# RomanJuranek/librectify

Measured on AMD Instinct MI355X. Metric: Mpix/s end-to-end (detect+VP) on 4K frames, batch call of 64 frames, 5 in flight, higher is better.
Workload: dtype f32

## Files before the change

librectify_amd/csrc/batch.hip:

```cpp
#include "host.h"

#include <cstdio>
#include <cstdlib>
#include <cstring>
#include <string>

namespace lramd {

static int find_groups_batch(lr_context* c, const void* d_images_, int format, size_t image_stride, const void* const* h_frames_,
                             int batch, int w, int h, int stride, float min_length, bool refine, int num_threads,
                             LineSegment* out, int capacity, int* n_lines, const RectificationConfig* cfg,
                             ImageTransform* transforms) {
    if (batch <= 0) return 0;
    const uint8_t* d_images = static_cast<const uint8_t*>(d_images_);
    const uint8_t* const* h_frames = reinterpret_cast<const uint8_t* const*>(h_frames_);
    const size_t bpp = (size_t)pix_bytes(format);
    if (bpp == 0) {
        set_error("unknown pixel format of the frames");
        return 1;
    }
    const int S = std::max(1, std::min(c->opt.batch_streams, batch));
    while ((int)c->workers.size() < S - 1) {
        lr_context* wc = nullptr;
        if (ctx_create(c->device, &wc)) return 1;
        c->workers.push_back(wc);
    }
    std::vector<lr_context*> lanes;
    lanes.push_back(c);
    for (int i = 0; i < S - 1; ++i) lanes.push_back(c->workers[i]);
    for (lr_context* l : lanes) {
        l->opt = c->opt;
        l->flood_log_min = S == 1 ? 0 : 32;
        l->flood_log_walk = S == 1 ? 0 : 24;
        l->flood_logbig_off = S > 1;
        l->flood_jit_sleep_us = S == 1 ? 0 : 20;
        static const bool sleep_env = std::getenv("LIBRECTIFY_LANES_SLEEP") != nullptr;
        l->sleep_in_wait = sleep_env && h_frames != nullptr;
    }
    const size_t npix = (size_t)w * h;
    int R = 0;
    bool any_pageable = false;
    std::vector<char> locked(h_frames ? (size_t)batch : 0, 0);
    if (h_frames) {
        if (w < 1 || h < 1) {
            set_error("upload: bad frame");
            return 1;
        }
        if ((stride < 0 ? -stride : stride) < w) {
            set_error("upload: |stride| smaller than the width");
            return 1;
        }
        for (int i = 0; i < batch; ++i) {
            if (h_frames[i] == nullptr) {
                set_error("upload: bad frame");
                return 1;
            }
        }
        for (int i = 0; i < batch; ++i) {
            locked[(size_t)i] = is_page_locked(h_frames[i]);
            any_pageable = any_pageable || !locked[(size_t)i];
        }
        static const int extra_env = std::getenv("LIBRECTIFY_RING_EXTRA") ? std::max(1, std::atoi(std::getenv("LIBRECTIFY_RING_EXTRA"))) : 0;
        const int by_bytes = (int)std::min<size_t>(64, ((size_t)2 << 30) / (npix * bpp));
        R = extra_env ? S + extra_env : std::max(S + 1, std::min(S + 6, by_bytes));
        R = std::min(batch, R);
        if (ensure_upload_ring(c, R, npix, any_pageable)) return 1;
    }
    std::vector<std::atomic<int>> enq(h_frames ? (size_t)batch : 0);
    std::vector<std::atomic<int>> slot_busy((size_t)R);
    struct SlotEdges {
        int r_lo = 0, r_hi = 0;
    };
    std::vector<SlotEdges> slot_edges((size_t)R);
    for (auto& a : enq) a.store(0, std::memory_order_relaxed);
    for (auto& a : slot_busy) a.store(0, std::memory_order_relaxed);
    static const bool lane_debug = std::getenv("LIBRECTIFY_LANE_DEBUG") != nullptr;
    constexpr size_t kBatchBand = (size_t)4 << 20;
    std::atomic<int> abort_all{0};
    std::string up_err;
    auto nap = [](int& spins) {
        if (++spins < 64) std::this_thread::yield();
        else std::this_thread::sleep_for(std::chrono::microseconds(30));
    };
    static const bool batch_stats = std::getenv("LIBRECTIFY_BATCH_STATS") != nullptr;
    std::atomic<long long> up_wait_us{0}, lane_wait_us{0}, lead_sum_us{0};
    std::atomic<int> late_frames{0};
    static const int register_threads = std::getenv("LIBRECTIFY_REGISTER_FRAMES") ? std::max(0, std::atoi(std::getenv("LIBRECTIFY_REGISTER_FRAMES"))) : 4;
    if (c->register_slow_calls > 0) --c->register_slow_calls;
    const bool reg_frames = register_threads > 0 && h_frames != nullptr && any_pageable && stride >= w && c->register_slow_calls == 0;
    const size_t row_bytes = (size_t)w * bpp, pitch = (size_t)(stride < 0 ? -stride : stride) * bpp;
    struct RegPlan {
        uintptr_t lo = 0, hi = 0;
        int r_lo = 0, r_hi = 0;
    };
    std::vector<RegPlan> plan(reg_frames ? (size_t)batch : 0);
    if (reg_frames) {
        constexpr uintptr_t kPage = 4096;
        for (int i = 0; i < batch; ++i) {
            RegPlan& p = plan[(size_t)i];
            const uintptr_t a = reinterpret_cast<uintptr_t>(h_frames[i]), e = a + (size_t)(h - 1) * pitch + row_bytes;
            const uintptr_t lo = (a + kPage - 1) / kPage * kPage, hi = e / kPage * kPage;
            if (hi <= lo) continue;
            const int r_lo = (int)((lo - a + pitch - 1) / pitch);
            const int r_hi = hi - a >= row_bytes ? (int)std::min<size_t>((size_t)h, (hi - a - row_bytes) / pitch + 1) : 0;
            if (r_hi - r_lo < h / 2) continue;
            bool apart = !locked[(size_t)i] && !c->batch_no_register;
            for (int j = 0; j < i && apart; ++j) {
                const RegPlan& q = plan[(size_t)j];
                apart = q.hi <= q.lo || q.hi <= lo || hi <= q.lo;
            }
            if (!apart) continue;
            p.lo = lo;
            p.hi = hi;
            p.r_lo = r_lo;
            p.r_hi = r_hi;
        }
    }
    std::atomic<int> reg_slow{0};
    std::vector<std::atomic<int>> reg_ready(reg_frames ? (size_t)batch : 0);
    for (auto& a : reg_ready) a.store(0, std::memory_order_relaxed);
    std::atomic<int> reg_next{0};
    std::vector<std::thread> reg_pool;
    if (reg_frames)
        for (int t = 0; t < register_threads; ++t)
            reg_pool.emplace_back([&]() {
                (void)hipSetDevice(c->device);
                bind_this_thread_near(c->device);
                for (int i = reg_next.fetch_add(1, std::memory_order_relaxed); i < batch && !abort_all.load(std::memory_order_relaxed);
                     i = reg_next.fetch_add(1, std::memory_order_relaxed)) {
                    if (reg_slow.load(std::memory_order_relaxed) >= 2) break;
                    int expect = 0;
                    if (!reg_ready[(size_t)i].compare_exchange_strong(expect, 3, std::memory_order_acq_rel)) continue;
                    int ok = 2;
                    const double t_r0 = now_ms();
                    const RegPlan& p = plan[(size_t)i];
                    if (p.hi > p.lo)
                        ok = hipHostRegister(reinterpret_cast<void*>(p.lo), p.hi - p.lo, hipHostRegisterDefault) == hipSuccess ? 1 : 2;
                    if (ok == 2) (void)hipGetLastError();
                    if (ok == 1 && (now_ms() - t_r0) * 6.0e6 > (double)(p.hi - p.lo)) reg_slow.fetch_add(1, std::memory_order_relaxed);
                    reg_ready[(size_t)i].store(ok, std::memory_order_release);
                }
            });
    const double t_call0 = now_ms();
    auto uploader = [&]() {
        if (hipSetDevice(c->device) != hipSuccess) {
            up_err = "hipSetDevice failed";
            abort_all.store(1);
            return;
        }
        if (any_pageable) bind_this_thread_near(c->device);
        StagingCrew crew;
        if (any_pageable) crew.start(c, staging_threads(num_threads, npix * bpp) - 1);
        for (int i = 0; i < batch; ++i) {
            int slot = -1, spins = 0;
            const double t_w0 = batch_stats ? now_ms() : 0.0;
            while (slot < 0 && !abort_all.load(std::memory_order_relaxed)) {
                for (int k = 0; k < R && slot < 0; ++k)
                    if (!slot_busy[(size_t)k].load(std::memory_order_acquire)) slot = k;
                if (slot < 0) nap(spins);
            }
            if (batch_stats) up_wait_us.fetch_add((long long)((now_ms() - t_w0) * 1e3));
            if (abort_all.load(std::memory_order_relaxed)) return;
            slot_busy[(size_t)slot].store(1, std::memory_order_relaxed);
            if (reg_frames) {
                int sp2 = 0;
                int expect = 0;
                if (!reg_ready[(size_t)i].compare_exchange_strong(expect, 2, std::memory_order_acq_rel))
                    while (reg_ready[(size_t)i].load(std::memory_order_acquire) == 3 && !abort_all.load(std::memory_order_relaxed)) nap(sp2);
            }
            const bool registered = reg_frames && reg_ready[(size_t)i].load(std::memory_order_acquire) == 1;
            uint8_t* stage = locked[(size_t)i] ? nullptr : reinterpret_cast<uint8_t*>(c->ring.stage[(size_t)slot].get());
            uint8_t* dimg = reinterpret_cast<uint8_t*>(c->ring.img[(size_t)slot].get());
            const double t_u0 = now_ms();
            Event e_dbg;
            if (lane_debug && e_dbg.create() == hipSuccess) (void)hipEventRecord(e_dbg, c->copy_stream);
            int up_rc = 0;
            if (registered) {
                const RegPlan& p = plan[(size_t)i];
                const uint8_t* f = h_frames[i];
                for (int r = 0; r < p.r_lo; ++r) std::memcpy(stage + (size_t)r * row_bytes, f + (size_t)r * pitch, row_bytes);
                for (int r = p.r_hi; r < h; ++r) std::memcpy(stage + (size_t)r * row_bytes, f + (size_t)r * pitch, row_bytes);
                slot_edges[(size_t)slot].r_lo = p.r_lo;
                slot_edges[(size_t)slot].r_hi = p.r_hi;
                {
                    const hipError_t e = pitch == row_bytes
                        ? hipMemcpyAsync(dimg + (size_t)p.r_lo * row_bytes, f + (size_t)p.r_lo * pitch, (size_t)(p.r_hi - p.r_lo) * row_bytes, hipMemcpyHostToDevice, c->copy_stream)
                        : hipMemcpy2DAsync(dimg + (size_t)p.r_lo * row_bytes, row_bytes, f + (size_t)p.r_lo * pitch, pitch, row_bytes, (size_t)(p.r_hi - p.r_lo), hipMemcpyHostToDevice, c->copy_stream);
                    if (e != hipSuccess) up_rc = 1;
                }
                if (up_rc) {
                    (void)hipGetLastError();
                    set_error("upload: transfer of a registered frame failed");
                }
            } else {
                slot_edges[(size_t)slot].r_hi = 0;
                up_rc = stage ? crew.run(dimg, stage, h_frames[i], w, h, stride, (int)bpp, c->copy_stream, kBatchBand, 1)
                              : upload_rows(c, dimg, nullptr, h_frames[i], w, h, stride, (int)bpp, 1, c->copy_stream);
            }
            if (up_rc || hipEventRecord(c->ring_ev[(size_t)slot], c->copy_stream) != hipSuccess) {
                up_err = get_error().empty() ? "upload failed" : get_error();
                abort_all.store(1);
                return;
            }
            enq[(size_t)i].store(slot + 1, std::memory_order_release);
            if (lane_debug) {
                const double t_u1 = now_ms();
                float dma = 0.f;
                if (e_dbg) {
                    (void)hipEventSynchronize(c->ring_ev[(size_t)slot]);
                    if (hipEventElapsedTime(&dma, e_dbg, c->ring_ev[(size_t)slot]) != hipSuccess) (void)hipGetLastError();
                }
                std::fprintf(stderr, "uploader frame %d: slot %d, waited %d naps for it, staged and enqueued in %.2f ms, on the link %.2f ms\n", i, slot, spins, t_u1 - t_u0, dma);
            }
        }
    };
    std::atomic<int> next_frame{0};
    std::vector<int> rc(S, 0);
    std::vector<std::string> err(S);
    auto work = [&](int si) {
        lr_context* l = lanes[si];
        auto fail = [&]() {
            rc[si] = 1;
            err[si] = get_error();
            abort_all.store(1);
        };
        if (si > 0 && hipSetDevice(c->device) != hipSuccess) {
            set_error("hipSetDevice failed");
            return fail();
        }
        for (int b = next_frame.fetch_add(1, std::memory_order_relaxed); b < batch; b = next_frame.fetch_add(1, std::memory_order_relaxed)) {
            const void* img = nullptr;
            int img_stride = stride, slot = -1;
            if (h_frames) {
                int spins = 0;
                const double t_w0 = batch_stats ? now_ms() : 0.0;
                while ((slot = enq[(size_t)b].load(std::memory_order_acquire) - 1) < 0 && !abort_all.load(std::memory_order_relaxed)) nap(spins);
                if (batch_stats) lane_wait_us.fetch_add((long long)((now_ms() - t_w0) * 1e3));
                if (slot < 0) return;
                if (hipStreamWaitEvent(l->stream, c->ring_ev[(size_t)slot], 0) != hipSuccess) {
                    set_error("hipStreamWaitEvent failed");
                    return fail();
                }
                img = c->ring.img[(size_t)slot].get();
                img_stride = w;
                const SlotEdges ed = slot_edges[(size_t)slot];
                if (ed.r_hi > 0) {
                    uint8_t* dimg = reinterpret_cast<uint8_t*>(c->ring.img[(size_t)slot].get());
                    const uint8_t* st = reinterpret_cast<const uint8_t*>(c->ring.stage[(size_t)slot].get());
                    hipError_t e = hipSuccess;
                    if (ed.r_lo > 0) e = hipMemcpyAsync(dimg, st, (size_t)ed.r_lo * row_bytes, hipMemcpyHostToDevice, l->stream);
                    if (e == hipSuccess && ed.r_hi < h)
                        e = hipMemcpyAsync(dimg + (size_t)ed.r_hi * row_bytes, st + (size_t)ed.r_hi * row_bytes, (size_t)(h - ed.r_hi) * row_bytes, hipMemcpyHostToDevice, l->stream);
                    if (e != hipSuccess) {
                        (void)hipGetLastError();
                        set_error("upload: transfer of a registered frame's first or last rows failed");
                        return fail();
                    }
                }
            } else {
                img = d_images + (size_t)b * image_stride * bpp;
            }
            std::vector<LineSegment> res;
            const double t_f0 = now_ms();
            if (ctx_find_groups_device(l, img, format, w, h, img_stride, min_length, refine, res)) return fail();
            if (batch_stats && h_frames && l->opt.timing_on) {
                float lead = 0.f;
                if (hipEventElapsedTime(&lead, c->ring_ev[(size_t)slot], l->ev[0]) == hipSuccess) {
                    lead_sum_us.fetch_add((long long)(lead * 1e3));
                    if (lead < 0.05f) late_frames.fetch_add(1);
                } else {
                    (void)hipGetLastError();
                }
            }
            if (lane_debug) {
                float lead = 0.f;
                if (h_frames && hipEventElapsedTime(&lead, c->ring_ev[(size_t)slot], l->ev[0]) != hipSuccess) (void)hipGetLastError();
                std::fprintf(stderr, "lane %d frame %d: enqueue %.2f ms, wait %.2f, whole call %.2f; device total %.2f; upload done %.2f ms before the first kernel\n",
                             si, b, l->host_ms[0], l->host_ms[2], now_ms() - t_f0, l->stage_ms[LR_T_TOTAL], lead);
            }
            if (h_frames) slot_busy[(size_t)slot].store(0, std::memory_order_release);
            const int n = (int)res.size();
            if (n_lines) n_lines[b] = n;
            if (out && capacity > 0)
                std::memcpy(out + (size_t)b * capacity, res.data(), sizeof(LineSegment) * (size_t)std::min(n, capacity));
            if (transforms) {
                const RectificationConfig def;
                transforms[b] = rectification_transform(res.data(), std::min(n, capacity > 0 ? capacity : n), w, h,
                                                        cfg ? *cfg : def);
            }
        }
    };
    std::vector<std::thread> th;
    if (h_frames) th.emplace_back(uploader);
    for (int si = 1; si < S; ++si) th.emplace_back(work, si);
    work(0);
    for (auto& t : th) t.join();
    if (batch_stats && h_frames)
        std::fprintf(stderr, "batch of %d frames: %.2f ms; the uploader waited %.2f ms for free device frames; the %d lanes waited %.2f ms in all for their frame's transfer to be enqueued\n",
                     batch, now_ms() - t_call0, up_wait_us.load() * 1e-3, S, lane_wait_us.load() * 1e-3);
    if (batch_stats && h_frames && c->opt.timing_on)
        std::fprintf(stderr, "   a frame's transfer was finished %.3f ms (mean) before its first kernel started; %d of %d frames started within 0.05 ms of it (they waited for the link)\n",
                     lead_sum_us.load() * 1e-3 / batch, late_frames.load(), batch);
    if (h_frames) (void)hipStreamSynchronize(c->copy_stream);
    for (auto& t : reg_pool) t.join();
    if (reg_slow.load() >= 2) c->register_slow_calls = 32;
    if (reg_frames)
        for (int i = 0; i < batch; ++i)
            if (reg_ready[(size_t)i].load(std::memory_order_acquire) == 1 && hipHostUnregister(reinterpret_cast<void*>(plan[(size_t)i].lo)) != hipSuccess)
                (void)hipGetLastError();
    for (lr_context* l : lanes) l->sleep_in_wait = false;
    c->flood_logbig_off = false;
    c->flood_log_min = c->flood_log_walk = 0;
    c->flood_jit_sleep_us = 0;
    for (int si = 0; si < S; ++si)
        if (rc[si]) {
            set_error(err[si]);
            return 1;
        }
    if (abort_all.load()) {
        set_error(up_err.empty() ? "batch: upload failed" : up_err);
        return 1;
    }
    return 0;
}

int ctx_find_groups_batch_device(lr_context* c, const void* d_images, int format, size_t image_stride, int batch, int w, int h,
                                 int stride, float min_length, bool refine, LineSegment* out, int capacity, int* n_lines,
                                 const RectificationConfig* cfg, ImageTransform* transforms) {
    return find_groups_batch(c, d_images, format, image_stride, nullptr, batch, w, h, stride, min_length, refine, -1, out,
                             capacity, n_lines, cfg, transforms);
}

int ctx_find_groups_batch_host(lr_context* c, const void* const* frames, int format, int batch, int w, int h, int stride,
                               float min_length, bool refine, int num_threads, LineSegment* out, int capacity,
                               int* n_lines, const RectificationConfig* cfg, ImageTransform* transforms) {
    return find_groups_batch(c, nullptr, format, 0, frames, batch, w, h, stride, min_length, refine, num_threads, out, capacity,
                             n_lines, cfg, transforms);
}

int ctx_find_groups_batch_host_multi(lr_context* c, const int* devices, int n_devices, const void* const* frames, int format, int batch,
                                     int w, int h, int stride, float min_length, bool refine, int num_threads,
                                     LineSegment* out, int capacity, int* n_lines, const RectificationConfig* cfg,
                                     ImageTransform* transforms) {
    if (batch <= 0) return 0;
    if (n_devices <= 0 || devices == nullptr) {
        set_error("multi-device batch: empty device list");
        return 1;
    }
    int ndev = 0;
    if (hipGetDeviceCount(&ndev) != hipSuccess) ndev = 0;
    for (int i = 0; i < n_devices; ++i)
        if (devices[i] < 0 || devices[i] >= ndev) {
            set_error("multi-device batch: device index out of range");
            return 1;
        }
    if ((int)c->peers.size() > n_devices) {
        for (size_t i = (size_t)n_devices; i < c->peers.size(); ++i) ctx_destroy(c->peers[i]);
        c->peers.resize((size_t)n_devices);
    }
    c->peers.resize((size_t)n_devices, nullptr);
    for (int i = 0; i < n_devices; ++i) {
        if (c->peers[(size_t)i] && c->peers[(size_t)i]->device != devices[i]) {
            ctx_destroy(c->peers[(size_t)i]);
            c->peers[(size_t)i] = nullptr;
        }
        if (!c->peers[(size_t)i] && ctx_create(devices[i], &c->peers[(size_t)i])) {
            (void)hipSetDevice(c->device);
            return 1;
        }
        c->peers[(size_t)i]->opt = c->opt;
    }
    const int per = (batch + n_devices - 1) / n_devices;
    bool blocks_apart = true;
    if (const size_t fbpp = (size_t)pix_bytes(format)) {
        const size_t span = (size_t)(h - 1) * (size_t)(stride < 0 ? -stride : stride) * fbpp + (size_t)w * fbpp;
        for (int i = 0; i < batch && blocks_apart && w > 0 && h > 0; ++i)
            for (int j = (i / per + 1) * per; j < batch && blocks_apart; ++j) {
                if (!frames[i] || !frames[j]) continue;
                const uintptr_t a = reinterpret_cast<uintptr_t>(frames[i]) - (stride < 0 ? (size_t)(h - 1) * (size_t)(-stride) * fbpp : 0);
                const uintptr_t b = reinterpret_cast<uintptr_t>(frames[j]) - (stride < 0 ? (size_t)(h - 1) * (size_t)(-stride) * fbpp : 0);
                blocks_apart = a + span <= b || b + span <= a;
            }
    }
    for (lr_context* p : c->peers) p->batch_no_register = !blocks_apart;
    std::vector<int> rc((size_t)n_devices, 0);
    std::vector<std::string> err((size_t)n_devices);
    auto run = [&](int i) {
        const int b0 = std::min(batch, i * per), b1 = std::min(batch, b0 + per);
        if (b1 <= b0) return;
        lr_context* p = c->peers[(size_t)i];
        if (hipSetDevice(p->device) != hipSuccess) {
            rc[(size_t)i] = 1;
            err[(size_t)i] = "hipSetDevice failed";
            return;
        }
        const int nt = num_threads > 1 ? std::max(2, num_threads / std::min(n_devices, (batch + per - 1) / per)) : num_threads;
        if (ctx_find_groups_batch_host(p, frames + b0, format, b1 - b0, w, h, stride, min_length, refine, nt,
                                       out ? out + (size_t)b0 * capacity : nullptr, capacity, n_lines ? n_lines + b0 : nullptr, cfg,
                                       transforms ? transforms + b0 : nullptr)) {
            rc[(size_t)i] = 1;
            err[(size_t)i] = get_error();
        }
    };
    std::vector<std::thread> th;
    for (int i = 1; i < n_devices; ++i) th.emplace_back(run, i);
    run(0);
    for (auto& t : th) t.join();
    (void)hipSetDevice(c->device);
    for (int i = 0; i < n_devices; ++i)
        if (rc[(size_t)i]) {
            set_error("device list entry " + std::to_string(i) + " (device " + std::to_string(devices[i]) + "): " + err[(size_t)i]);
            return 1;
        }
    return 0;
}

}
```

librectify_amd/csrc/common.h:

```cpp
#pragma once
#include <hip/hip_runtime.h>

#include <cstdint>
#include <string>

#include "../../include/librectify_amd.h"

namespace lramd {

constexpr float kEps = 1e-6f;
constexpr int kMaxModels = 4;
constexpr int kMaxPeelModels = 5;
constexpr float kInlierDeg = 2.0f;
constexpr float kGarbageDeg = 4.0f;
constexpr int kRansacMaxIter = 10000;
constexpr int kEdgeKernelSize = 2;
constexpr float kEdgeKernelSigma = 1.0f;
constexpr int kSeedDist = 2;
constexpr float kSeedRatio = 0.95f;
constexpr float kTraceTolerance = 0.25f;
constexpr float kLineMaxErr = 2.0f;
constexpr float kLineMinLength = 5.f;
constexpr int kComponentMinSize = 5;
constexpr int kBins = 8;

struct FilterConsts {
    float d[5];
    float g[5];
    float st[kBins];
    float ct[kBins];
};

struct BinTrig {
    float st[kBins];
    float ct[kBins];
};

constexpr uint32_t kLabelFree = 0xFFFFFFFFu;

__host__ __device__ inline float directional(float dx, float dy, float s, float c) {
    return fabsf(fmaf(dx, s, dy * c));
}

__host__ __device__ inline uint64_t splitmix64(uint64_t x) {
    x += 0x9E3779B97F4A7C15ull;
    x = (x ^ (x >> 30)) * 0xBF58476D1CE4E5B9ull;
    x = (x ^ (x >> 27)) * 0x94D049BB133111EBull;
    return x ^ (x >> 31);
}
__host__ __device__ inline void sample_pair(uint64_t seed, uint32_t round, uint32_t iter, uint32_t n, uint32_t& a,
                                            uint32_t& b) {
    const uint64_t z = splitmix64(seed ^ splitmix64(((uint64_t)round << 32) | iter));
    const uint32_t u1 = (uint32_t)z, u2 = (uint32_t)(z >> 32);
    const uint32_t i = (uint32_t)(((uint64_t)u1 * n) >> 32);
    uint32_t j = (uint32_t)(((uint64_t)u2 * (n - 1)) >> 32);
    if (j >= i) ++j;
    a = i < j ? i : j;
    b = i < j ? j : i;
}

void set_error(const std::string& msg);

#define LR_HIP(expr)                                                                                     \
    do {                                                                                                 \
        hipError_t _e = (expr);                                                                          \
        if (_e != hipSuccess) {                                                                          \
            (void)hipGetLastError();        \
            ::lramd::set_error(std::string(#expr) + ": " + hipGetErrorString(_e) + " (" + __FILE__ + ":" + \
                               std::to_string(__LINE__) + ")");                                          \
            return 1;                                                                                    \
        }                                                                                                \
    } while (0)

inline int pix_bytes(int format) { return format == LR_PIX_U8 ? 1 : format == LR_PIX_U8X3 ? 3 : format == LR_PIX_F32 ? 4 : 0; }
int launch_filter(const void* img, int format, int w, int h, int stride, const FilterConsts& fc, float* dx, float* dy,
                  uint8_t* dmask, uint64_t* cand, uint32_t* cand_count, uint32_t* tile_max, hipStream_t s);
int filter_band_rows();
int filter_band_last_row(int by);
int launch_filter_rows(const void* img, int format, int w, int h, int stride, const FilterConsts& fc, float* dx, float* dy,
                       uint8_t* dmask, uint64_t* cand, uint32_t* cand_count, uint32_t* tile_max, int by_begin, int by_end,
                       hipStream_t s);
struct FilterGeom {
    int n_tiles;
    int cand_cap;
};
FilterGeom filter_geometry(int w, int h);

size_t seeds_temp_bytes(int n_tiles, size_t max_seeds);
int launch_seed_select(const uint64_t* cand, const uint32_t* cand_count, const uint32_t* tile_max, int n_tiles,
                       int cand_cap, float seed_keep_ratio, float* maxmag, uint32_t* tile_pass, uint32_t* tile_off, uint64_t* keys,
                       uint32_t key_cap, uint32_t* n_seeds, uint32_t frame_tag, hipStream_t s);
int launch_seed_order(uint64_t* keys, uint64_t* keys_alt, const uint32_t* n_seeds, uint32_t cap, const float* dx, const float* dy,
                      BinTrig trig, float trace_tolerance, int32_t* seed_idx, int32_t* seed_bin, float* seed_thr, hipStream_t s);

int launch_label_init(uint32_t* label, size_t n, hipStream_t s);
int launch_flood_ordered(const float* dx, const float* dy, const uint8_t* dmask, int w, int h, const int32_t* seed_idx,
                         const int32_t* seed_bin, const float* seed_thr, const uint32_t* d_n_seeds, uint32_t seed_cap,
                         BinTrig trig, uint32_t* label, int32_t* seed_size, int32_t* queue, hipStream_t s);

constexpr size_t kFloodHandWords = 1024;
struct FloodBuffers {
    uint32_t* blocked = nullptr;
    uint32_t* count = nullptr;
    uint32_t* flags = nullptr;
    uint8_t* state = nullptr;
    uint8_t* tier = nullptr;
    uint32_t* blk = nullptr;
    uint32_t* act_a = nullptr;
    uint32_t* act_b = nullptr;
    uint32_t* ctrl = nullptr;
    uint8_t* dirty = nullptr;
    uint32_t* big_list = nullptr;
    uint32_t* handover = nullptr;
    bool rewalk_logs = false;
    uint32_t* rewalk_list = nullptr;
    int log_min_tiles = 0, log_walk_tiles = 0;
    bool giant_hold = false;
    bool giant_step = true;
    void* giant_mask = nullptr;
    uint32_t* giant_parent = nullptr;
    bool log_sweep = false;
    bool rewalk_big = false;
    uint32_t log_seeds = 0, log_cap = 0;
    uint32_t* log_off = nullptr;
    uint32_t* log_len = nullptr;
    uint32_t* log_buf = nullptr;
    void* slab_ring = nullptr;
    void* slab_hash = nullptr;
    uint32_t n_slabs = 0, slab_ring_cap = 0, slab_hash_cap = 0;
    int win_first_shift = 0, win_growth = 2;
    int win_hold_pct = 80;
    bool partial_commits = true;
    bool second_tier = true;
    bool second_tier_from_start = true;
    bool hold_from_start = false;
    bool staged_from_start = false;
    int blind_rounds = 10;
    uint32_t* host_progress = nullptr;
    bool calm_hint = false;
    uint32_t* host_ctrl = nullptr;
    int jit_first = 0;
    int jit_sleep_us = 0;
    uint32_t big_cap_override = 0;
    uint32_t team_tile_cap = 0;
};
struct FloodFrame {
    const float* dx;
    const float* dy;
    const uint8_t* dmask;
    int w, h;
    const int32_t* seed_idx;
    const int32_t* seed_bin;
    const float* seed_thr;
    const uint32_t* d_n_seeds;
    uint32_t seed_cap;
    BinTrig trig;
    uint32_t* label;
    int32_t* seed_size;
    int32_t* queue;
};
struct FloodProgress {
    int enqueued = 0;
    bool use_big = false;
    int win_growth = 2;
    bool sizes_known = false;
    uint32_t max_flood = 0;
};
constexpr int kFloodCtrlWords = 56;
int flood_enqueue(const FloodBuffers& B, const FloodFrame& F, FloodProgress* P, uint32_t* h_ctrl, hipStream_t s);
int flood_finish(const FloodBuffers& B, const FloodFrame& F, FloodProgress* P, uint32_t* h_ctrl, int* rounds_out,
                 uint32_t* tiers_out ,
                 bool* extra, hipStream_t s);

size_t fit_temp_bytes(size_t max_pixels, uint32_t max_segments);
struct HugeSort {
    uint32_t* tab = nullptr;
    uint32_t* list = nullptr;
    uint32_t* jobs = nullptr;
    uint32_t max = 0;
};
int launch_component_offsets(const int32_t* seed_size, const uint32_t* d_n_seeds, uint32_t seed_cap, int min_size,
                             uint32_t* comp_rank, uint32_t* comp_seed, uint32_t* comp_off,
                             uint32_t* totals , uint32_t* large_list, uint32_t large_cap,
                             uint32_t* n_large, void* temp, size_t temp_bytes, uint32_t frame_tag, uint32_t* cursor, const HugeSort& hs,
                             hipStream_t s);
int launch_component_scatter(const uint32_t* label, size_t npix, const uint32_t* comp_rank, const uint32_t* comp_off,
                             uint32_t* cursor, uint32_t* px, const HugeSort& hs, uint32_t* n_large, bool with_huge, hipStream_t s);
int launch_component_sort(const uint32_t* px_in, uint32_t* px_out, const uint32_t* comp_off, const uint32_t* d_n_comp,
                          uint32_t comp_cap, const uint32_t* large_list, uint32_t large_cap, const uint32_t* n_large,
                          uint32_t* scratch, const uint32_t* cursor, const HugeSort& hs, bool with_huge, hipStream_t s);
int launch_fit(const uint32_t* px_sorted, const uint32_t* px_unsorted, const uint32_t* comp_off, const uint32_t* comp_seed, const uint32_t* d_n_comp,
               uint32_t comp_cap, const int32_t* seed_bin, const float* dx, const float* dy, int w, BinTrig trig,
               float* scratch_w, LineSegment* out, const uint32_t* cursor, const HugeSort& hs, const uint32_t* n_large, bool with_huge,
               hipStream_t s);

struct PencilSoA {
    const float* ax;
    const float* ay;
    const float* dx;
    const float* dy;
    const float* len;
    const float* hx;
    const float* hy;
    const float* hz;
};
constexpr int kRansacBestSlots = 32;
int launch_ransac_score(PencilSoA m, uint32_t n, float tol, float degeneracy_tol, uint32_t n_iter, uint64_t seed,
                        uint32_t round, unsigned long long* best_slots, uint32_t* host_best, hipStream_t s);
int launch_ransac_score_dev(PencilSoA m, const uint32_t* gctl, int max_models, float tol, float degeneracy_tol,
                            uint32_t n_iter, uint64_t seed, unsigned long long* best_slots, hipStream_t s);

struct PencilTable {
    float* ax;
    float* ay;
    float* dx;
    float* dy;
    float* len;
    float* hx;
    float* hy;
    float* hz;
    uint32_t* orig;
    PencilSoA soa() const { return PencilSoA{ax, ay, dx, dy, len, hx, hy, hz}; }
};
enum {
    kGcLines = 0,
    kGcRemaining = 1,
    kGcRound = 2,
    kGcActive = 3,
    kGcBestIter0 = 4,
    kGcWords = 8,
};
int launch_filter_lines(const LineSegment* raw, const uint32_t* d_n_raw, uint32_t raw_cap, float min_length,
                        LineSegment* out, uint32_t* gctl, float* gnorm, const PencilTable* all, const PencilTable* round0,
                        hipStream_t s);
int launch_lines_bbox(LineSegment* lines, uint32_t n, uint32_t* gctl, float* gnorm, hipStream_t s);
int launch_pencil_model(const LineSegment* lines, const uint32_t* gctl, const float* gnorm, PencilTable all,
                        PencilTable round0, uint32_t line_cap, hipStream_t s);
int launch_peel(PencilTable cur, PencilTable nxt, PencilTable all, unsigned long long* best_slots, uint64_t seed,
                float tol, float garbage_tol, int max_models, uint32_t* gctl, float* stage4 ,
                LineSegment* lines, float* models,
                const uint32_t* counts, uint32_t cap_lines, void* gather_block ,
                hipStream_t s);
int launch_cht_accumulate(PencilSoA m, uint32_t n, int d, unsigned long long* acc, hipStream_t s);
int launch_cht_votes(PencilSoA m, const uint32_t* idx, uint32_t n, int d, unsigned long long* acc, bool subtract,
                     unsigned long long* n_votes, hipStream_t s);
int launch_cht_peak(const unsigned long long* acc, int d, uint32_t* out3, hipStream_t s);
int launch_refine_pairs(const void* seg, uint32_t n, void* edges, uint32_t* n_edges, uint32_t cap, hipStream_t s);
int launch_prosac_count(PencilSoA m, uint32_t n, float tol, float degeneracy_tol, const uint32_t* sa,
                        const uint32_t* sb, uint32_t n_hyp, uint32_t* counts, hipStream_t s);
int launch_prosac_flags(PencilSoA m, uint32_t n, float px, float py, float pz, float tol, uint8_t* flags, hipStream_t s);
int launch_prosac_records(PencilSoA m, uint32_t n, const uint32_t* sa, const uint32_t* sb, const uint32_t* counts,
                          uint32_t n_hyp, uint32_t best_in, float tol, uint32_t* rec, uint32_t cap, uint8_t* flags, hipStream_t s);
int launch_ht_weights(PencilSoA m, uint32_t n, const int32_t* pa, const int32_t* pb, int n_pairs, int ht, float* peak,
                      float* weights, hipStream_t s);

}
```

librectify_amd/csrc/context.hip:

```cpp
#include "host.h"

#include <cmath>
#include <cstdlib>

#ifndef M_PI
#define M_PI 3.14159265358979323846
#endif

lr_context::lr_context() = default;
lr_context::~lr_context() = default;

namespace lramd {

namespace {

thread_local std::string g_error;

void gauss_deriv_factors(int size, float sigma, float* d, float* g) {
    const int n = 2 * size + 1;
    for (int t = 0; t < n; ++t) {
        const float x = float(t - size);
        const float a = float(2 * M_PI * std::pow(sigma, 4.0f));
        const float e = std::exp(-std::pow(x, 2.0f) / (2 * std::pow(sigma, 2.0f)));
        d[t] = x / a * e;
        g[t] = e;
    }
}

void init_constants(lr_context* c) {
    gauss_deriv_factors(kEdgeKernelSize, kEdgeKernelSigma, c->fconsts.d, c->fconsts.g);
    for (int b = 0; b < kBins; ++b) {
        const float theta = float(b * M_PI) / kBins;
        c->trig.st[b] = std::sin(theta);
        c->trig.ct[b] = std::cos(theta);
        c->fconsts.st[b] = c->trig.st[b];
        c->fconsts.ct[b] = c->trig.ct[b];
    }
    c->seed_keep_ratio = 1 - std::max(std::min(kSeedRatio, 1.f), 0.f);
}

}

void set_error(const std::string& msg) { g_error = msg; }
const std::string& get_error() { return g_error; }

int ctx_trim(lr_context* c, bool frames_too) {
    LR_HIP(hipSetDevice(c->device));
    LR_HIP(hipStreamSynchronize(c->stream));
    if (c->copy_stream) LR_HIP(hipStreamSynchronize(c->copy_stream));
    c->ws = Workspace{};
    c->flood = FloodStore{};
    if (frames_too) {
        c->frames = FrameSlots{};
        c->ring.drop();
        c->prep = PrepareSpans{};
    }
    c->small_frames = 0;
    c->w = c->h = 0;
    c->seed_cap = 0;
    c->flood_hold_hint = c->flood_staged_hint = c->flood_calm_hint = false;
    c->flood_staged_streak = 0;
    for (bool& v : c->stage_valid) v = false;
    if (frames_too)
        for (lr_context* wc : c->workers)
            if (ctx_trim(wc, true)) return 1;
    return 0;
}

int ctx_ensure_image_capacity(lr_context* c, int w, int h) {
    const size_t npix = (size_t)w * h;
    if (c->w != 0 && (c->w != w || c->h != h)) {
        c->flood_hold_hint = false;
        c->flood_staged_hint = false;
        c->flood_calm_hint = false;
        c->flood_staged_streak = 0;
    }
    const FilterGeom fg = filter_geometry(w, h);
    const int ntiles = fg.n_tiles;
    if (c->ws.cap_pix != 0 && npix * 4 <= c->ws.cap_pix) {
        if (++c->small_frames >= 8 && ctx_trim(c, false)) return 1;
    } else {
        c->small_frames = 0;
    }
    if (npix <= c->ws.cap_pix && ntiles <= c->ws.cap_tiles) return 0;
    LR_HIP(hipStreamSynchronize(c->stream));
    const size_t cp = std::max(npix, c->ws.cap_pix);
    const int ct = std::max(ntiles, c->ws.cap_tiles);
    const size_t tile_off_words = std::max(ct, 2);
    Workspace& s = c->ws;
    s.cap_pix = 0;
    s.cap_tiles = 0;
    if (s.dx.grow(cp) || s.dy.grow(cp) || s.dmask.grow(cp + 16) || s.cand.grow((size_t)ct * fg.cand_cap) || s.cand_count.grow(ct) ||
        s.tile_max.grow(ct) || s.tile_pass.grow(ct) || s.tile_off.grow(tile_off_words) || s.keys_a.grow(cp) || s.keys_b.grow(cp) ||
        s.seed_idx.grow(cp) || s.seed_bin.grow(cp) || s.seed_thr.grow(cp) || s.seed_size.grow(cp) || s.label.grow(cp) ||
        s.queue.grow(cp) || s.comp_rank.grow(cp) || s.comp_seed.grow(cp) || s.comp_off.grow(cp + 1) || s.cursor.grow(cp) ||
        s.px_a.grow(cp) || s.px_b.grow(cp) || s.scratch_w.grow(cp) || s.d_lines.grow(cp / 6 + 16) || s.comp_large.grow(cp / 64 + 16))
        return 1;
    LR_HIP(hipMemsetAsync(s.tile_off, 0, tile_off_words * sizeof(uint32_t), c->stream));
    {
        const size_t nb = (cp + 16383) >> 14;
        const uint32_t max = 256;
        if (s.huge_tab.grow(max * nb) || s.huge_jobs.grow(4 * max * nb) || s.huge_list.grow(max)) return 1;
        s.huge = HugeSort{s.huge_tab, s.huge_list, s.huge_jobs, max};
        LR_HIP(hipMemsetAsync(s.huge.tab, 0, max * nb * sizeof(uint32_t), c->stream));
    }
    const size_t tb = std::max(seeds_temp_bytes(ct, cp), fit_temp_bytes(cp, (uint32_t)std::min<size_t>(cp / 6 + 16, 0xFFFFFFFFu)));
    if (s.temp.grow(tb)) return 1;
    LR_HIP(hipMemsetAsync(s.temp, 0, tb, c->stream));
    s.cap_pix = cp;
    s.cap_tiles = ct;
    return 0;
}

template <class T, class P>
static int grow_into(DeviceBuffer<T>& own, P*& raw, size_t count) {
    raw = nullptr;
    if (own.grow(count)) return 1;
    raw = own.get();
    return 0;
}

static int ensure_flood_slabs(lr_context* c) {
    FloodBuffers& f = c->flood.fb;
    static const bool giant_step_off = std::getenv("LIBRECTIFY_FLOOD_GIANT_STEP") && std::atoi(std::getenv("LIBRECTIFY_FLOOD_GIANT_STEP")) == 0;
    uint32_t want = (c->opt.flood_mode == 1 && c->opt.flood_giant_step && !giant_step_off) ? 16u : 128u;
    if (const char* e = std::getenv("LIBRECTIFY_FLOOD_SLABS")) want = (uint32_t)std::max(1, std::atoi(e));
    if (f.slab_ring && f.n_slabs >= want) return 0;
    LR_HIP(hipStreamSynchronize(c->stream));
    f.n_slabs = want;
    f.slab_ring_cap = 1u << 14;
    f.slab_hash_cap = 1u << 16;
    if (grow_into(c->flood.slab_ring, f.slab_ring, (size_t)f.n_slabs * f.slab_ring_cap) ||
        grow_into(c->flood.slab_hash, f.slab_hash, (size_t)f.n_slabs * f.slab_hash_cap * 2))
        return 1;
    LR_HIP(hipMemsetAsync(f.slab_hash, 0, (size_t)f.n_slabs * f.slab_hash_cap * 32, c->stream));
    if (f.ctrl) LR_HIP(hipMemsetAsync(f.ctrl, 0, kFloodCtrlWords * sizeof(uint32_t), c->stream));
    return 0;
}

int ensure_flood_buffers(lr_context* c) {
    FloodStore& o = c->flood;
    FloodBuffers& f = o.fb;
    if (c->flood.cap_seeds >= c->ws.cap_pix && f.ctrl) return ensure_flood_slabs(c);
    LR_HIP(hipStreamSynchronize(c->stream));
    const size_t cs = c->ws.cap_pix;
    if (grow_into(o.blocked, f.blocked, cs) || grow_into(o.count, f.count, cs) || grow_into(o.flags, f.flags, cs) ||
        grow_into(o.state, f.state, cs) || grow_into(o.tier, f.tier, cs) || grow_into(o.blk, f.blk, cs) ||
        grow_into(o.act_a, f.act_a, cs) || grow_into(o.act_b, f.act_b, cs) || grow_into(o.ctrl, f.ctrl, kFloodCtrlWords) ||
        grow_into(o.big_list, f.big_list, 8192) || grow_into(o.handover, f.handover, 8192 * kFloodHandWords) ||
        grow_into(o.dirty, f.dirty, cs / 256 + 16) ||
        grow_into(o.giant_mask, f.giant_mask, cs / 16 + 64))
        return 1;
    constexpr size_t kLogCapDiv = 8;
    f.log_seeds = (uint32_t)std::min<size_t>(std::max<size_t>(cs / 16, 4096), cs);
    f.log_cap = (uint32_t)std::min<size_t>(std::max<size_t>(cs / kLogCapDiv, 65536), 1u << 28);
    if (grow_into(o.rewalk_list, f.rewalk_list, 8192) || grow_into(o.log_off, f.log_off, f.log_seeds) ||
        grow_into(o.log_len, f.log_len, f.log_seeds) || grow_into(o.log_buf, f.log_buf, (size_t)f.log_cap * 3))
        return 1;
    LR_HIP(hipMemsetAsync(f.ctrl, 0, kFloodCtrlWords * sizeof(uint32_t), c->stream));
    o.cap_seeds = cs;
    return ensure_flood_slabs(c);
}


int ctx_ensure_ransac_capacity(lr_context* c, size_t n_lines) {
    if (8 * n_lines <= c->model.cap()) return 0;
    LR_HIP(hipStreamSynchronize(c->stream));
    return c->model.grow(8 * std::max<size_t>(n_lines, 4096));
}

int ensure_group_capacity(lr_context* c, size_t n_lines) {
    if (n_lines > c->cap_glines) {
        LR_HIP(hipStreamSynchronize(c->stream));
        const size_t cl = std::max<size_t>(n_lines, 4096);
        c->cap_glines = 0;
        if (c->d_tables.grow(3 * 8 * cl) || c->d_orig.grow(3 * cl) || c->d_inl.grow(4 * cl)) return 1;
        c->cap_glines = cl;
    }
    if (n_lines > c->d_flines.cap()) {
        LR_HIP(hipStreamSynchronize(c->stream));
        if (c->d_flines.grow(n_lines + 16)) return 1;
    }
    return 0;
}

int ctx_create(int device, lr_context** out) {
    int ndev = 0;
    if (hipGetDeviceCount(&ndev) != hipSuccess || ndev <= 0) {
        set_error("no HIP device available: librectify_amd has no CPU fallback");
        return 1;
    }
    if (device < 0 || device >= ndev) {
        set_error("device index out of range");
        return 1;
    }
    LR_HIP(hipSetDevice(device));
    lr_context* c = new lr_context();
    c->device = device;
    if (hipStreamCreateWithFlags(c->stream.put(), hipStreamNonBlocking) != hipSuccess) {
        delete c;
        set_error("hipStreamCreate failed");
        return 1;
    }
    {
        static const int fail_at = std::getenv("LIBRECTIFY_TEST_CREATE_FAIL") ? std::atoi(std::getenv("LIBRECTIFY_TEST_CREATE_FAIL")) : 0;
        int n_alloc = 0;
        hipError_t bad = hipSuccess;
        const char* what = "";
        auto check = [&](hipError_t e, const char* name) {
            if (++n_alloc == fail_at) e = hipErrorOutOfMemory;
            if (e != hipSuccess && bad == hipSuccess) {
                bad = e;
                what = name;
            }
        };
        for (auto& e : c->ev) check(e.create(), "hipEventCreate");
        check(c->ev_wait.create(hipEventBlockingSync | hipEventDisableTiming), "hipEventCreate");
        static const bool lane_debug = std::getenv("LIBRECTIFY_LANE_DEBUG") != nullptr;
        for (auto& e : c->ev_up) check(e.create(lane_debug ? hipEventDefault : hipEventDisableTiming), "hipEventCreate");
        check(c->maxmag.alloc(1), "hipMalloc(maxmag)");
        check(c->d_counts.alloc(64), "hipMalloc(counts)");
        check(c->d_gctl.alloc(kGcWords), "hipMalloc(peeling control block)");
        check(c->d_gnorm.alloc(4), "hipMalloc(normalisation)");
        check(c->d_models.alloc(64), "hipMalloc(models)");
        check(c->d_best_slots.alloc(kRansacBestSlots), "hipMalloc(best slots)");
        check(c->h_counts.alloc(128), "hipHostMalloc(counts)");
        check(c->h_best.alloc(2), "hipHostMalloc(best)");
        if (bad == hipSuccess) check(hipMemset(c->d_models, 0, 64 * sizeof(float)), "hipMemset(models)");
        if (bad == hipSuccess) check(hipMemset(c->d_counts, 0, 64 * sizeof(uint32_t)), "hipMemset(counts)");
        if (bad == hipSuccess) check(hipMemset(c->d_best_slots, 0, kRansacBestSlots * sizeof(unsigned long long)), "hipMemset(best slots)");
        if (bad != hipSuccess) {
            (void)hipGetLastError();
            const std::string msg = std::string("lr_context_create: ") + what + " failed: " + hipGetErrorString(bad);
            ctx_destroy(c);
            set_error(msg);
            return 1;
        }
    }
    init_constants(c);
    const char* env = std::getenv("LIBRECTIFY_SEED");
    c->opt.ransac_seed = env ? std::strtoull(env, nullptr, 0) : 0ull;
    c->opt.timing_on = std::getenv("LIBRECTIFY_STAGE_TIMES") != nullptr;
    if (const char* e = std::getenv("LIBRECTIFY_FLOOD_LOGS")) c->opt.flood_logs = std::atoi(e) != 0;
    *out = c;
    return 0;
}

void ctx_destroy(lr_context* c) {
    if (!c) return;
    for (lr_context* wc : c->workers) ctx_destroy(wc);
    for (lr_context* pc : c->peers) ctx_destroy(pc);
    (void)hipSetDevice(c->device);
    (void)hipStreamSynchronize(c->stream);
    if (c->copy_stream) (void)hipStreamSynchronize(c->copy_stream);
    c->crew.reset();
    delete c;
}

}
```

librectify_amd/csrc/frame.hip:

```cpp
#include "host.h"

#include <cstdio>
#include <cstdlib>
#include <cstring>

namespace lramd {


namespace {

uint32_t round_up(uint32_t v, uint32_t m) { return (v + m - 1) / m * m; }

uint32_t initial_seed_cap(size_t npix) {
    return (uint32_t)std::min<size_t>(npix, std::max<size_t>(round_up((uint32_t)(npix / 32), 1024), 4096));
}

uint32_t line_cap_for(const lr_context* c) {
    return (uint32_t)std::min<size_t>(c->seed_cap, c->ws.cap_pix / 6 + 16);
}


PencilTable table_of(lr_context* c, int which) {
    const size_t cl = c->cap_glines;
    float* b = c->d_tables + (size_t)which * 8 * cl;
    return PencilTable{b, b + cl, b + 2 * cl, b + 3 * cl, b + 4 * cl, b + 5 * cl, b + 6 * cl, b + 7 * cl,
                       c->d_orig + (size_t)which * cl};
}

int ensure_result_block(lr_context* c, size_t lines) {
    if (lines <= c->res_lines_cap && c->h_res) return 0;
    LR_HIP(hipStreamSynchronize(c->stream));
    if (c->h_res.grow(kResHeaderBytes + lines * sizeof(LineSegment))) return 1;
    c->res_lines_cap = lines;
    return 0;
}

FloodBuffers flood_buffers_for(lr_context* c) {
    FloodBuffers fbuf = c->flood.fb;
    if (c->opt.flood_mode >= 2 && c->opt.flood_mode <= 4) fbuf.second_tier = false;
    fbuf.second_tier_from_start = c->flood_big_hint;
    fbuf.hold_from_start = c->flood_hold_hint;
    fbuf.staged_from_start = c->flood_staged_hint;
    if (c->opt.flood_mode == 2) fbuf.n_slabs = 0;
    if (c->opt.flood_mode == 3) fbuf.n_slabs = 2;
    if (c->opt.flood_mode == 5) {
        fbuf.n_slabs = 0;
        fbuf.big_cap_override = 1;
    }
    if (c->opt.flood_mode == 6) fbuf.team_tile_cap = 200;
    if (c->opt.flood_mode == 7) {
        fbuf.team_tile_cap = 200;
        fbuf.n_slabs = 0;
    }
    static const bool partial_off = std::getenv("LIBRECTIFY_FLOOD_PARTIAL") && std::atoi(std::getenv("LIBRECTIFY_FLOOD_PARTIAL")) == 0;
    fbuf.partial_commits = !partial_off && c->opt.flood_partial;
    fbuf.rewalk_logs = c->opt.flood_logs;
    fbuf.log_sweep = c->opt.flood_log_sweep;
    fbuf.log_min_tiles = c->flood_log_min;
    fbuf.log_walk_tiles = c->flood_log_walk;
    fbuf.giant_hold = c->opt.flood_mode == 1;
    static const bool giant_step_off = std::getenv("LIBRECTIFY_FLOOD_GIANT_STEP") && std::atoi(std::getenv("LIBRECTIFY_FLOOD_GIANT_STEP")) == 0;
    fbuf.giant_step = !giant_step_off && c->opt.flood_giant_step;
    fbuf.giant_parent = reinterpret_cast<uint32_t*>(c->ws.queue.get());
    fbuf.rewalk_big = c->flood_logbig_hint && !c->flood_logbig_off;
    if (c->opt.flood_staged) fbuf.win_first_shift = 3;
    fbuf.blind_rounds = c->flood_rounds_hint;
    static const bool jit_off = std::getenv("LIBRECTIFY_FLOOD_JIT") && std::atoi(std::getenv("LIBRECTIFY_FLOOD_JIT")) == 0;
    static_assert(16 + kFloodCtrlWords <= 72, "the control block's copy ends where the report word begins");
    fbuf.host_progress = c->h_counts + 72;
    fbuf.host_ctrl = c->h_counts + 16;
    static const int calm_hint_env = std::getenv("LIBRECTIFY_FLOOD_CALM_HINT") ? std::atoi(std::getenv("LIBRECTIFY_FLOOD_CALM_HINT")) : 1;
    fbuf.calm_hint = calm_hint_env != 0 && c->flood_calm_hint;
    fbuf.jit_sleep_us = c->flood_jit_sleep_us;
    constexpr int kJitFirstMax = 4;
    fbuf.jit_first = (c->opt.flood_jit && !jit_off) ? std::min(c->flood_rounds_last > 0 ? std::max(c->flood_rounds_last - 1, 2) : 3, kJitFirstMax) : 0;
    return fbuf;
}

FloodFrame flood_frame_for(lr_context* c) {
    return FloodFrame{c->ws.dx, c->ws.dy, c->ws.dmask, c->w, c->h, c->ws.seed_idx, c->ws.seed_bin, c->ws.seed_thr,
                      c->d_counts + kCntSeeds, c->seed_cap, c->trig, c->ws.label, c->ws.seed_size, c->ws.queue};
}

int prepare_frame(lr_context* c, int w, int h) {
    LR_HIP(hipSetDevice(c->device));
    if (w < 5 || h < 5) {
        set_error("image smaller than the 5x5 filter");
        return 1;
    }
    if (ctx_ensure_image_capacity(c, w, h)) return 1;
    if (c->w != w || c->h != h || c->seed_cap == 0) c->seed_cap = initial_seed_cap((size_t)w * h);
    if (c->seed_cap_once) {
        c->seed_cap = (uint32_t)std::min<size_t>((size_t)w * h, c->seed_cap_once);
        c->seed_cap_once = 0;
    }
    c->w = w;
    c->h = h;
    c->n_seeds = c->n_comp = c->n_px = 0;
    c->dmask_consumed = false;
    for (bool& v : c->stage_valid) v = false;
    return 0;
}

int enqueue_filter(lr_context* c, const void* d_image, int format, int w, int h, int stride) {
    if (prepare_frame(c, w, h)) return 1;
    const size_t bpp = (size_t)pix_bytes(format);
    if (bpp == 0 || d_image == nullptr || stride < w) {
        set_error(bpp == 0 ? "unknown pixel format of the frames" : "launch_filter: bad geometry");
        return 1;
    }
    const size_t npix = (size_t)w * h;
    if (format == LR_PIX_U8X3) {
        if (npix >= ((size_t)1 << 29)) {
            set_error("launch_filter: image larger than 2^29 pixels is not supported (seed key packs index in 29 bits)");
            return 1;
        }
        if (c->frames.luma.cap() < npix) {
            LR_HIP(hipStreamSynchronize(c->stream));
            if (c->frames.luma.grow(npix)) return 1;
        }
        if (ctx_prepare_frames(c, d_image, 0, 1, w, h, (size_t)stride * bpp, LR_PIX_U8X3, c->frames.luma.get(), 0, w, h, (size_t)w * sizeof(float)))
            return 1;
        d_image = c->frames.luma.get();
        format = LR_PIX_F32;
        stride = w;
    }
    const size_t fbpp = (size_t)pix_bytes(format);
    if (stride > w && (uint64_t)w * (uint64_t)h < (1ull << 29) &&
        ((uint64_t)(h - 1) * (uint64_t)stride + (uint64_t)w) * fbpp >= (1ull << 32)) {
        if (c->frames.packed.cap() < npix) {
            LR_HIP(hipStreamSynchronize(c->stream));
            if (c->frames.packed.grow(npix)) return 1;
        }
        LR_HIP(hipMemcpy2DAsync(c->frames.packed, (size_t)w * fbpp, d_image, (size_t)stride * fbpp,
                                (size_t)w * fbpp, (size_t)h, hipMemcpyDeviceToDevice, c->stream));
        d_image = c->frames.packed;
        stride = w;
    }
    if (c->opt.timing_on) LR_HIP(hipEventRecord(c->ev[0], c->stream));
    if (launch_filter(d_image, format, w, h, stride, c->fconsts, c->ws.dx, c->ws.dy, c->ws.dmask, c->ws.cand, c->ws.cand_count, c->ws.tile_max,
                      c->stream))
        return 1;
    if (c->opt.timing_on) LR_HIP(hipEventRecord(c->ev[1], c->stream));
    return 0;
}

int enqueue_seeds(lr_context* c) {
    const FilterGeom fg = filter_geometry(c->w, c->h);
    if (launch_seed_select(c->ws.cand, c->ws.cand_count, c->ws.tile_max, fg.n_tiles, fg.cand_cap, c->seed_keep_ratio, c->maxmag,
                           c->ws.tile_pass, c->ws.tile_off, c->ws.keys_a, c->seed_cap, c->d_counts + kCntSeeds, ++c->select_tag ? c->select_tag : ++c->select_tag,
                           c->stream))
        return 1;
    if (launch_seed_order(c->ws.keys_a, c->ws.keys_b, c->d_counts + kCntSeeds, c->seed_cap, c->ws.dx, c->ws.dy, c->trig, kTraceTolerance,
                          c->ws.seed_idx, c->ws.seed_bin, c->ws.seed_thr, c->stream))
        return 1;
    if (c->opt.timing_on) LR_HIP(hipEventRecord(c->ev[2], c->stream));
    return 0;
}

int enqueue_flood(lr_context* c) {
    const size_t npix = (size_t)c->w * c->h;
    c->flood_rounds = 1;
    if (c->opt.flood_mode == 0) {
        if (launch_label_init(c->ws.label, npix, c->stream)) return 1;
        if (launch_flood_ordered(c->ws.dx, c->ws.dy, c->ws.dmask, c->w, c->h, c->ws.seed_idx, c->ws.seed_bin, c->ws.seed_thr,
                                 c->d_counts + kCntSeeds, c->seed_cap, c->trig, c->ws.label, c->ws.seed_size, c->ws.queue, c->stream))
            return 1;
    } else {
        if (ensure_flood_buffers(c)) return 1;
        if (flood_enqueue(flood_buffers_for(c), flood_frame_for(c), &c->flood_prog, c->h_counts + 16, c->stream)) return 1;
        c->stage_valid[0] = c->stage_valid[1] = false;
        c->dmask_consumed = true;
    }
    if (c->opt.timing_on) LR_HIP(hipEventRecord(c->ev[3], c->stream));
    return 0;
}

int finish_flood(lr_context* c, bool* extra) {
    *extra = false;
    if (c->opt.flood_mode == 0) return 0;
    if (flood_finish(flood_buffers_for(c), flood_frame_for(c), &c->flood_prog, c->h_counts + 16, &c->flood_rounds,
                     c->flood_tiers, extra, c->stream))
        return 1;
    static const bool call_debug = std::getenv("LIBRECTIFY_CALL_DEBUG") != nullptr;
    if (call_debug)
        std::fprintf(stderr, "flood: %d rounds, %u walks in the second tier, %u of them long, hold-back phase %u (started with it: %d)\n",
                     c->flood_rounds, c->flood_tiers[0], c->flood_tiers[8], c->flood_tiers[3], (int)c->flood_hold_hint);
    c->flood_logbig_hint = c->flood_tiers[0] > 0;
    c->flood_calm_hint = c->flood_tiers[0] == 0 && c->flood_tiers[1] == 0 && c->flood_tiers[15] == 0;
    c->flood_big_hint = true;
    c->flood_hold_hint = c->flood_tiers[3] != 0 && c->flood_tiers[8] >= 16;
    constexpr uint32_t kStagedKeep = 64;
    c->flood_staged_hint = c->flood_tiers[14] != 0 && (!c->flood_staged_hint || c->flood_tiers[0] >= kStagedKeep);
    c->flood_staged_streak = c->flood_staged_hint ? c->flood_staged_streak + 1 : 0;
    if (c->flood_staged_streak >= 16) {
        c->flood_staged_hint = false;
        c->flood_staged_streak = 0;
    }
    if (c->flood_staged_hint) c->flood_hold_hint = false;

    c->flood_rounds_hint = std::max(std::max(c->flood_rounds + 2, 6), c->flood_rounds_hint - 1);
    c->flood_rounds_last = c->flood_rounds;
    return 0;
}

int enqueue_fit(lr_context* c) {
    const size_t npix = (size_t)c->w * c->h;
    const uint32_t comp_cap = line_cap_for(c);
    const bool with_huge = !(c->opt.flood_mode != 0 && c->flood_prog.sizes_known && c->flood_prog.max_flood <= (1u << 14));
    if (launch_component_offsets(c->ws.seed_size, c->d_counts + kCntSeeds, c->seed_cap, kComponentMinSize, c->ws.comp_rank,
                                 c->ws.comp_seed, c->ws.comp_off, c->d_counts + kCntComp, c->ws.comp_large,
                                 (uint32_t)(c->ws.cap_pix / 64 + 16), c->d_counts + kCntLarge, c->ws.temp, c->ws.temp.cap(), ++c->fit_tag ? c->fit_tag : ++c->fit_tag, c->ws.cursor,
                                 with_huge ? c->ws.huge : HugeSort{}, c->stream))
        return 1;
    if (launch_component_scatter(c->ws.label, npix, c->ws.comp_rank, c->ws.comp_off, c->ws.cursor, c->ws.px_a, c->ws.huge, c->d_counts + kCntLarge, with_huge,
                                 c->stream))
        return 1;
    if (launch_component_sort(c->ws.px_a, c->ws.px_b, c->ws.comp_off, c->d_counts + kCntComp, comp_cap, c->ws.comp_large,
                              (uint32_t)(c->ws.cap_pix / 64 + 16), c->d_counts + kCntLarge, reinterpret_cast<uint32_t*>(c->ws.keys_b.get()),
                              c->ws.cursor, c->ws.huge, with_huge, c->stream))
        return 1;
    static const bool fit_debug = std::getenv("LIBRECTIFY_FIT_DEBUG") != nullptr;
    if (fit_debug) {
        uint32_t cnt[16];
        LR_HIP(hipStreamSynchronize(c->stream));
        LR_HIP(hipMemcpy(cnt, c->d_counts, sizeof(cnt), hipMemcpyDeviceToHost));
        std::fprintf(stderr, "fit: with_huge %d (sizes known %d, largest flood %u); seeds %u comps %u px %u; lists: %u of 65..1024 px, %u longer, %u huge in %u buckets; counter %u\n",
                     (int)with_huge, (int)c->flood_prog.sizes_known, c->flood_prog.max_flood, cnt[0], cnt[1], cnt[2], cnt[4], cnt[5], cnt[6], cnt[7], cnt[10]);
        const uint32_t nj = std::min<uint32_t>(cnt[7], 6);
        std::vector<uint32_t> jobs(4 * nj + 4);
        if (nj) LR_HIP(hipMemcpy(jobs.data(), c->ws.huge.jobs, nj * 16, hipMemcpyDeviceToHost));
        for (uint32_t j = 0; j < nj; ++j) std::fprintf(stderr, "   bucket job %u: start %u, %u px, table word %u\n", j, jobs[4 * j], jobs[4 * j + 1], jobs[4 * j + 2]);
    }
    if (launch_fit(c->ws.px_b, c->ws.px_a, c->ws.comp_off, c->ws.comp_seed, c->d_counts + kCntComp, comp_cap, c->ws.seed_bin, c->ws.dx, c->ws.dy, c->w,
                   c->trig, c->ws.scratch_w, c->ws.d_lines, c->ws.cursor, c->ws.huge, c->d_counts + kCntLarge, with_huge, c->stream))
        return 1;
    if (c->opt.timing_on) LR_HIP(hipEventRecord(c->ev[4], c->stream));
    return 0;
}

}

int enqueue_groups(lr_context* c, uint32_t line_cap, int max_models, float inlier_deg, float garbage_deg, int n_iter,
                   uint64_t seed, bool model_done, bool gather) {
    if (max_models > kMaxPeelModels) {
        set_error("estimate_line_pencils: max_models above " + std::to_string(kMaxPeelModels) + " (the reference uses 4, config.h:25)");
        return 1;
    }
    const float tol = cos_threshold(inlier_deg), garbage_tol = cos_threshold(garbage_deg);
    const PencilTable all = table_of(c, 0);
    PencilTable tab[2] = {table_of(c, 1), table_of(c, 2)};
    if (!model_done && launch_pencil_model(c->d_flines, c->d_gctl, c->d_gnorm, all, tab[0], line_cap, c->stream)) return 1;
    const float degeneracy_tol = 0.05f;
    for (int k = 0; k < max_models; ++k) {
        if (n_iter > 0 &&
            launch_ransac_score_dev(tab[k & 1].soa(), c->d_gctl, max_models, tol, degeneracy_tol, (uint32_t)n_iter, seed,
                                    c->d_best_slots, c->stream))
            return 1;
        const bool last = gather && k == max_models - 1;
        if (launch_peel(tab[k & 1], tab[(k + 1) & 1], all, c->d_best_slots, seed, tol, garbage_tol,
                        max_models, c->d_gctl, c->d_inl, c->d_flines, c->d_models, c->d_counts,
                        (uint32_t)std::min<size_t>(c->res_lines_cap, c->d_flines.cap()), last ? c->h_res.get() : nullptr, c->stream))
            return 1;
    }
    return 0;
}

namespace {

void record_stage_times(lr_context* c, bool with_groups) {
    if (!c->opt.timing_on) return;
    float ms = 0.f;
    (void)hipEventElapsedTime(&ms, c->ev[0], c->ev[1]);
    c->stage_ms[LR_T_FILTER] = ms;
    c->stage_ms[LR_T_FILTER_KERNEL] = ms;
    (void)hipEventElapsedTime(&ms, c->ev[1], c->ev[2]);
    c->stage_ms[LR_T_SEEDS] = ms;
    (void)hipEventElapsedTime(&ms, c->ev[2], c->ev[3]);
    c->stage_ms[LR_T_FLOOD] = ms;
    (void)hipEventElapsedTime(&ms, c->ev[3], c->ev[4]);
    c->stage_ms[LR_T_FIT] = ms;
    if (with_groups) {
        (void)hipEventElapsedTime(&ms, c->ev[5], c->ev[6]);
        c->stage_ms[LR_T_RANSAC] = ms;
        (void)hipEventElapsedTime(&ms, c->ev[0], c->ev[6]);
        c->stage_ms[LR_T_TOTAL] = ms;
    }
}

void adapt_seed_cap(lr_context* c, uint32_t n_seeds) {
    const size_t npix = (size_t)c->w * c->h;
    if (n_seeds > c->seed_cap)
        c->seed_cap = (uint32_t)std::min<size_t>(npix, std::max<uint32_t>(4096, round_up(n_seeds * 2u, 1024)));
    else if (n_seeds < c->seed_cap / 3 || n_seeds > c->seed_cap / 5 * 4)
        c->seed_cap = (uint32_t)std::min<size_t>(npix, std::max<uint32_t>(4096, round_up(n_seeds + n_seeds / 2, 1024)));
}

}

struct TimingOn {
    lr_context* c;
    bool was;
    explicit TimingOn(lr_context* ctx) : c(ctx), was(ctx->opt.timing_on) { c->opt.timing_on = true; }
    ~TimingOn() { c->opt.timing_on = was; }
};

int ctx_stage_filter(lr_context* c, const float* d_image, int w, int h, int stride) {
    TimingOn t(c);
    if (enqueue_filter(c, d_image, LR_PIX_F32, w, h, stride)) return 1;
    c->stage_valid[0] = true;
    return 0;
}

int ctx_stage_seeds(lr_context* c) {
    if (!c->stage_valid[0]) {
        set_error("lr_stage_seeds: run lr_stage_filter first");
        return 1;
    }
    TimingOn t(c);
    for (int attempt = 0;; ++attempt) {
        if (enqueue_seeds(c)) return 1;
        LR_HIP(hipMemcpyAsync(c->h_counts, c->d_counts, sizeof(uint32_t), hipMemcpyDeviceToHost, c->stream));
        LR_HIP(hipStreamSynchronize(c->stream));
        c->n_seeds = c->h_counts[0];
        if (c->n_seeds <= c->seed_cap) break;
        if (attempt > 0) {
            set_error("seed count exceeds the sort capacity twice");
            return 1;
        }
        adapt_seed_cap(c, c->n_seeds);
    }
    c->stage_valid[1] = true;
    return 0;
}

int ctx_stage_flood(lr_context* c) {
    if (!c->stage_valid[1]) {
        set_error(c->dmask_consumed ? "lr_stage_flood: the previous flood consumed the filter output; run lr_stage_filter and lr_stage_seeds again"
                                    : "lr_stage_flood: run lr_stage_seeds first");
        return 1;
    }
    TimingOn t(c);
    if (enqueue_flood(c)) return 1;
    LR_HIP(hipStreamSynchronize(c->stream));
    bool extra;
    if (finish_flood(c, &extra)) return 1;
    c->stage_valid[2] = true;
    return 0;
}

int ctx_stage_fit(lr_context* c, std::vector<LineSegment>& out) {
    if (!c->stage_valid[2]) {
        set_error("lr_stage_fit: run lr_stage_flood first");
        return 1;
    }
    out.clear();
    TimingOn t(c);
    if (enqueue_fit(c)) return 1;
    LR_HIP(hipMemcpyAsync(c->h_counts, c->d_counts, 8 * sizeof(uint32_t), hipMemcpyDeviceToHost, c->stream));
    LR_HIP(hipStreamSynchronize(c->stream));
    c->n_comp = c->h_counts[kCntComp];
    c->n_px = c->h_counts[kCntPx];
    if (c->n_comp > 0) {
        out.resize(c->n_comp);
        LR_HIP(hipMemcpyAsync(out.data(), c->ws.d_lines, (size_t)c->n_comp * sizeof(LineSegment), hipMemcpyDeviceToHost,
                              c->stream));
        LR_HIP(hipStreamSynchronize(c->stream));
    }
    c->stage_valid[3] = true;
    record_stage_times(c, false);
    return 0;
}

int ctx_detect(lr_context* c, const float* d_image, int w, int h, int stride, std::vector<LineSegment>& raw) {
    if (ctx_stage_filter(c, d_image, w, h, stride)) return 1;
    if (ctx_stage_seeds(c)) return 1;
    if (ctx_stage_flood(c)) return 1;
    return ctx_stage_fit(c, raw);
}

int run_frame(lr_context* c, const void* d_image, int format, int w, int h, int stride, float min_length, bool refine,
              std::vector<LineSegment>& out, bool filter_enqueued) {
    out.clear();
    const double t_begin = now_ms();
    const bool fused = !refine && c->opt.estimator == 0;
    const int n_iter = c->opt.ransac_iters;
    auto groups_after_fit = [&]() -> int {
        const uint32_t lc = line_cap_for(c);
        if (ensure_group_capacity(c, lc)) return 1;
        if (ensure_result_block(c, std::max<size_t>(c->res_lines_cap, 4096))) return 1;
        if (c->opt.timing_on) LR_HIP(hipEventRecord(c->ev[5], c->stream));
        const PencilTable all = table_of(c, 0), round0 = table_of(c, 1);
        if (launch_filter_lines(c->ws.d_lines, c->d_counts + kCntComp, lc, min_length, c->d_flines, c->d_gctl, c->d_gnorm, &all, &round0,
                                c->stream))
            return 1;
        static_assert(kMaxModels >= 1 && kGcWords == 8 && kResHeaderBytes == 256, "the last peeling round carries the result block (peel_kernel)");
        if (enqueue_groups(c, lc, kMaxModels, kInlierDeg, kGarbageDeg, n_iter, c->opt.ransac_seed, true, true)) return 1;
        if (c->opt.timing_on) LR_HIP(hipEventRecord(c->ev[6], c->stream));
        return 0;
    };
    auto after_fit = [&]() -> int {
        if (fused) return groups_after_fit();
        LR_HIP(hipMemcpyAsync(c->h_counts, c->d_counts, 8 * sizeof(uint32_t), hipMemcpyDeviceToHost, c->stream));
        return 0;
    };
    c->frame_laps = 0;
    for (int attempt = 0;; ++attempt) {
        c->frame_laps += 1;
        if (!(filter_enqueued && attempt == 0) && enqueue_filter(c, d_image, format, w, h, stride)) return 1;
        if (enqueue_seeds(c)) return 1;
        if (enqueue_flood(c)) return 1;
        if (enqueue_fit(c)) return 1;
        if (after_fit()) return 1;
        const double t_enq = now_ms();
        const double t_pre = now_ms();
        if (c->sleep_in_wait) {
            LR_HIP(hipEventRecord(c->ev_wait, c->stream));
            LR_HIP(hipEventSynchronize(c->ev_wait));
        } else {
            LR_HIP(hipStreamSynchronize(c->stream));
        }
        c->host_ms[0] = t_enq - t_begin;
        c->host_ms[1] = t_pre - t_enq;
        c->host_ms[2] = now_ms() - t_pre;
        const uint32_t* cnt = fused ? reinterpret_cast<const uint32_t*>(c->h_res.get()) : c->h_counts.get();
        c->n_seeds = cnt[kCntSeeds];
        if (c->n_seeds <= c->seed_cap) break;
        if (attempt > 0) {
            set_error("seed count exceeds the sort capacity twice");
            return 1;
        }
        adapt_seed_cap(c, c->n_seeds);
    }
    bool extra = false;
    if (finish_flood(c, &extra)) return 1;
    if (extra) {
        c->frame_laps += 1;
        if (enqueue_fit(c)) return 1;
        if (after_fit()) return 1;
        LR_HIP(hipStreamSynchronize(c->stream));
    }
    const uint32_t* cnt = fused ? reinterpret_cast<const uint32_t*>(c->h_res.get()) : c->h_counts.get();
    c->n_comp = cnt[kCntComp];
    c->n_px = cnt[kCntPx];
    adapt_seed_cap(c, c->n_seeds);
    c->stage_valid[0] = c->stage_valid[1] = false;
    c->stage_valid[2] = c->stage_valid[3] = true;
    if (fused) {
        const uint32_t* gctl = reinterpret_cast<const uint32_t*>(c->h_res + 32);
        const size_t n = gctl[kGcLines];
        out.resize(n);
        const size_t have = std::min<size_t>(n, c->res_lines_cap);
        if (have) std::memcpy(out.data(), c->h_res + kResHeaderBytes, have * sizeof(LineSegment));
        if (n > have) {
            LR_HIP(hipMemcpyAsync(out.data() + have, c->d_flines + have, (n - have) * sizeof(LineSegment),
                                  hipMemcpyDeviceToHost, c->stream));
            LR_HIP(hipStreamSynchronize(c->stream));
            if (ensure_result_block(c, round_up((uint32_t)(n + n / 2), 1024))) return 1;
        }
        record_stage_times(c, true);
#ifdef LR_PEEL_TIMING
        {
            const float* tm = reinterpret_cast<const float*>(c->h_res + 64) + 16;
            for (int r = 0; r < 4; ++r)
                std::fprintf(stderr, "peel round %d: best %.1f us, inliers %.1f, sums %.1f, jacobi %.1f, verdict %.1f\n", r,
                             tm[r * 5], tm[r * 5 + 1], tm[r * 5 + 2], tm[r * 5 + 3], tm[r * 5 + 4]);
        }
#endif
        return 0;
    }
    std::vector<LineSegment> raw(c->n_comp);
    if (c->n_comp) {
        LR_HIP(hipMemcpyAsync(raw.data(), c->ws.d_lines, (size_t)c->n_comp * sizeof(LineSegment), hipMemcpyDeviceToHost,
                              c->stream));
        LR_HIP(hipStreamSynchronize(c->stream));
    }
    record_stage_times(c, false);
    if (raw.size() < 2) return 0;
    if (refine && ctx_refine(c, raw)) return 1;
    std::vector<LineSegment> filtered = filter_lines(raw, min_length);
    if (filtered.empty()) return 0;
    if (c->opt.timing_on) LR_HIP(hipEventRecord(c->ev[5], c->stream));
    if (c->opt.estimator == 1) {
        if (ctx_estimate_line_pencils_prosac(c, filtered, kMaxModels, kInlierDeg, kGarbageDeg, c->opt.prosac_T_N,
                                             c->opt.ransac_seed))
            return 1;
    } else if (c->opt.estimator == 2) {
        if (ctx_estimate_line_pencils_direct(c, filtered, kMaxModels, kInlierDeg, kGarbageDeg)) return 1;
    } else if (c->opt.estimator == 3) {
        if (ctx_estimate_line_pencils_cht(c, filtered, kMaxModels, kInlierDeg, kGarbageDeg, c->opt.cht_d, nullptr)) return 1;
    } else if (ctx_estimate_line_pencils(c, filtered, kMaxModels, kInlierDeg, kGarbageDeg, n_iter, c->opt.ransac_seed)) {
        return 1;
    }
    if (c->opt.timing_on) LR_HIP(hipEventRecord(c->ev[6], c->stream));
    LR_HIP(hipStreamSynchronize(c->stream));
    record_stage_times(c, true);
    out.swap(filtered);
    return 0;
}

int ctx_find_groups_device(lr_context* c, const void* d_image, int format, int w, int h, int stride, float min_length, bool refine,
                           std::vector<LineSegment>& out) {
    return run_frame(c, d_image, format, w, h, stride, min_length, refine, out);
}

int ctx_find_groups_host(lr_context* c, const void* buffer_, int format, int w, int h, int stride, float min_length, bool refine,
                         int num_threads, std::vector<LineSegment>& out) {
    const uint8_t* buffer = static_cast<const uint8_t*>(buffer_);
    const int bpp = pix_bytes(format);
    if (bpp == 0) {
        set_error("unknown pixel format of the frames");
        return 1;
    }
    const double t_call = now_ms();
    LR_HIP(hipSetDevice(c->device));
    if (w < 5 || h < 5 || buffer == nullptr) {
        set_error("image smaller than the 5x5 filter");
        return 1;
    }
    if ((stride < 0 ? -stride : stride) < w) {
        set_error("upload: |stride| smaller than the width");
        return 1;
    }
    if (ensure_copy_stream(c)) return 1;
    hipStream_t up = c->copy_stream;
    const size_t npix = (size_t)w * h;
    const int slot = 0;
    uint8_t* stage = nullptr;
    {
        float* stage_f = nullptr;
        if (ensure_frame_slot(c, slot, npix, !is_page_locked(buffer), &stage_f)) return 1;
        stage = reinterpret_cast<uint8_t*>(stage_f);
    }
    if (prepare_frame(c, w, h)) return 1;
    struct DrainOnError {
        lr_context* c;
        hipStream_t up;
        bool ok = false;
        ~DrainOnError() {
            if (ok) return;
            (void)hipStreamSynchronize(up);
            (void)hipStreamSynchronize(c->stream);
            (void)hipGetLastError();
        }
    } drain{c, up};
    const uint8_t* src = buffer;
    int sstride = stride;
    if (sstride < 0) {
        src = buffer + (std::ptrdiff_t)(h - 1) * sstride * bpp;
        sstride = -sstride;
    }
    const size_t row_bytes = (size_t)w * bpp, pitch = (size_t)sstride * bpp;
    const bool follow = format != LR_PIX_U8X3;
    static const size_t band_bytes = std::getenv("LIBRECTIFY_UPLOAD_BAND_KB") ? (size_t)std::max(64, std::atoi(std::getenv("LIBRECTIFY_UPLOAD_BAND_KB"))) << 10 : (size_t)4 << 20;
    static const bool band_env = std::getenv("LIBRECTIFY_UPLOAD_BAND_KB") != nullptr;
    int rpb = (int)std::max<size_t>(1, ((stage == nullptr && !band_env) ? (size_t)h * row_bytes : band_bytes) / row_bytes);
    if ((h + rpb - 1) / rpb > StagingCrew::kMaxBands) rpb = (h + StagingCrew::kMaxBands - 1) / StagingCrew::kMaxBands;
    const int n_bands = (h + rpb - 1) / rpb;
    while ((int)c->band_ev.size() < n_bands) {
        Event e;
        if (e.ensure(hipEventDisableTiming)) return 1;
        c->band_ev.push_back(std::move(e));
    }
    uint8_t* dst = reinterpret_cast<uint8_t*>(c->frames.slot[slot].get());
    const int fb = filter_band_rows(), band_rows = (h + fb - 1) / fb;
    int by_next = 0;
    auto filter_after_band = [&](int k) -> int {
        LR_HIP(hipStreamWaitEvent(c->stream, c->band_ev[(size_t)k], 0));
        if (!follow) return 0;
        const int last_row = std::min(h, (k + 1) * rpb) - 1;
        int by_end = by_next;
        while (by_end < band_rows && std::min(h - 1, filter_band_last_row(by_end)) <= last_row) ++by_end;
        if (k == n_bands - 1) by_end = band_rows;
        if (launch_filter_rows(dst, format, w, h, w, c->fconsts, c->ws.dx, c->ws.dy, c->ws.dmask, c->ws.cand, c->ws.cand_count, c->ws.tile_max, by_next,
                               by_end, c->stream))
            return 1;
        by_next = by_end;
        return 0;
    };
    if (follow && c->opt.timing_on) LR_HIP(hipEventRecord(c->ev[0], c->stream));
    const int T = stage ? staging_threads(num_threads, npix * bpp) : 1;
    if (T <= 1) {
        for (int k = 0; k < n_bands; ++k) {
            const int r0 = k * rpb, r1 = std::min(h, r0 + rpb);
            if (stage) {
                if (sstride == w) std::memcpy(stage + (size_t)r0 * row_bytes, src + (size_t)r0 * pitch, (size_t)(r1 - r0) * row_bytes);
                else
                    for (int r = r0; r < r1; ++r) std::memcpy(stage + (size_t)r * row_bytes, src + (size_t)r * pitch, row_bytes);
                LR_HIP(hipMemcpyAsync(dst + (size_t)r0 * row_bytes, stage + (size_t)r0 * row_bytes, (size_t)(r1 - r0) * row_bytes,
                                      hipMemcpyHostToDevice, up));
            } else if (sstride == w) {
                LR_HIP(hipMemcpyAsync(dst + (size_t)r0 * row_bytes, src + (size_t)r0 * row_bytes, (size_t)(r1 - r0) * row_bytes,
                                      hipMemcpyHostToDevice, up));
            } else {
                LR_HIP(hipMemcpy2DAsync(dst + (size_t)r0 * row_bytes, row_bytes, src + (size_t)r0 * pitch, pitch,
                                        row_bytes, (size_t)(r1 - r0), hipMemcpyHostToDevice, up));
            }
            LR_HIP(hipEventRecord(c->band_ev[(size_t)k], up));
            if (filter_after_band(k)) return 1;
        }
    } else {
        if (!c->crew || c->crew_helpers != T) {
            c->crew.reset();
            c->crew.reset(new StagingCrew());
            c->crew->start(c, T);
            c->crew_helpers = T;
        }
        StagingCrew* cr = c->crew.get();
        std::vector<std::atomic<int>> ready((size_t)n_bands);
        for (auto& a : ready) a.store(0, std::memory_order_relaxed);
        const uint32_t g = cr->begin(dst, stage, src, w, h, sstride, bpp, up, c->band_ev.data(), ready.data(), band_bytes);
        int rc = 0;
        for (int k = 0; k < n_bands && rc == 0; ++k) {
            int spins = 0, r;
            while ((r = ready[(size_t)k].load(std::memory_order_acquire)) == 0) {
                if ((cr->live.load(std::memory_order_acquire) == 0 || spins > 4096) && cr->work_one(g)) continue;
                if (++spins < 2048) std::this_thread::yield();
                else std::this_thread::sleep_for(std::chrono::microseconds(5));
            }
            if (r < 0 || filter_after_band(k)) rc = 1;
        }
        if (rc) cr->work(g);
        if (cr->finish() || rc) {
            if (get_error().empty()) set_error("upload: staging copy failed");
            return 1;
        }
    }
    if (follow && c->opt.timing_on) LR_HIP(hipEventRecord(c->ev[1], c->stream));
    LR_HIP(hipEventRecord(c->ev_up[slot], up));
    static const bool call_debug = std::getenv("LIBRECTIFY_CALL_DEBUG") != nullptr;
    const double t_up = now_ms();
    const int rc = run_frame(c, dst, format, w, h, w, min_length, refine, out, follow);
    drain.ok = rc == 0;
    if (call_debug)
        std::fprintf(stderr, "host frame: bands staged, sent and filter launched in %.3f ms; rest of the frame enqueued in %.3f ms; waited %.3f ms; "
                     "results out in %.3f ms; whole call %.3f ms\n", t_up - t_call, c->host_ms[0], c->host_ms[2],
                     now_ms() - t_up - c->host_ms[0] - c->host_ms[2], now_ms() - t_call);
    return rc;
}

}
```

librectify_amd/csrc/kernels_groups.hip:

```cpp
#include "common.h"

namespace lramd {
namespace {

constexpr int kWG = 1024;
constexpr int kWaves = kWG / 64;

__device__ __forceinline__ float wave_tree(float v) {
#pragma unroll
    for (int off = 32; off >= 1; off >>= 1) v = v + __shfl_xor(v, off);
    return v;
}

__device__ __forceinline__ uint32_t block_rank(bool flag, uint32_t* s_cnt, uint32_t& total) {
    const int lane = threadIdx.x & 63, wv = threadIdx.x >> 6;
    const uint64_t m = __ballot(flag);
    __syncthreads();
    if (lane == 0) s_cnt[wv] = (uint32_t)__popcll(m);
    __syncthreads();
    uint32_t before = 0, tot = 0;
#pragma unroll
    for (int i = 0; i < kWaves; ++i) {
        const uint32_t c = s_cnt[i];
        before += i < wv ? c : 0u;
        tot += c;
    }
    total = tot;
    return before + (uint32_t)__popcll(m & ((1ull << lane) - 1ull));
}

__device__ __forceinline__ void pencil_model_of(const LineSegment& l, uint32_t i, float cx, float cy, float sc, const PencilTable& all,
                                                const PencilTable& round0) {
    const float x1 = (l.x1 - cx) / sc, y1 = (l.y1 - cy) / sc, x2 = (l.x2 - cx) / sc, y2 = (l.y2 - cy) / sc;
    float hx = y1 * 1.f - 1.f * y2, hy = 1.f * x2 - x1 * 1.f, hz = x1 * y2 - y1 * x2;
    const float zz = (hx * hx + hy * hy) + hz * hz;
    if (zz > 0.0f) {
        const float nn = sqrtf(zz);
        hx = hx / nn;
        hy = hy / nn;
        hz = hz / nn;
    }
    const float ax = (x2 + x1) / 2, ay = (y2 + y1) / 2;
    const float dx = x2 - x1, dy = y2 - y1;
    const float len = sqrtf(dx * dx + dy * dy);
    const float ux = dx / len, uy = dy / len;
    all.ax[i] = ax; all.ay[i] = ay; all.dx[i] = ux; all.dy[i] = uy; all.len[i] = len;
    all.hx[i] = hx; all.hy[i] = hy; all.hz[i] = hz; all.orig[i] = i;
    round0.ax[i] = ax; round0.ay[i] = ay; round0.dx[i] = ux; round0.dy[i] = uy; round0.len[i] = len;
    round0.hx[i] = hx; round0.hy[i] = hy; round0.hz[i] = hz; round0.orig[i] = i;
}

__global__ __launch_bounds__(kWG) void filter_lines_kernel(const LineSegment* __restrict__ raw,
                                                           const uint32_t* __restrict__ n_raw_ptr, uint32_t raw_cap,
                                                           float min_length, LineSegment* __restrict__ out,
                                                           uint32_t* __restrict__ gctl, float* __restrict__ gnorm,
                                                           PencilTable all, PencilTable round0, uint32_t with_model) {
    constexpr int kFlB = 8;
    __shared__ uint32_t s_cnt[kFlB][kWaves];
    __shared__ float s_red[4][kWaves];
    const uint32_t n_raw = min(*n_raw_ptr, raw_cap);
    const float ml = fmaxf(min_length, kLineMinLength);
    const int lane = threadIdx.x & 63, wv = threadIdx.x >> 6;
    uint32_t base = 0;
    if (n_raw >= 2u) {
        for (uint32_t i0 = 0; i0 < n_raw; i0 += kWG * kFlB) {
            LineSegment l[kFlB];
            uint64_t m[kFlB];
#pragma unroll
            for (int b = 0; b < kFlB; ++b) {
                const uint32_t i = i0 + (uint32_t)b * kWG + threadIdx.x;
                l[b] = LineSegment{};
                if (i < n_raw) l[b] = raw[i];
            }
#pragma unroll
            for (int b = 0; b < kFlB; ++b) {
                const uint32_t i = i0 + (uint32_t)b * kWG + threadIdx.x;
                const float dx = l[b].x2 - l[b].x1, dy = l[b].y2 - l[b].y1;
                const bool keep = i < n_raw && sqrtf(dx * dx + dy * dy) > ml && l[b].err < kLineMaxErr;
                m[b] = __ballot(keep);
                if (lane == 0) s_cnt[b][wv] = (uint32_t)__popcll(m[b]);
            }
            __syncthreads();
#pragma unroll
            for (int b = 0; b < kFlB; ++b) {
                uint32_t before = 0, tot = 0;
#pragma unroll
                for (int w = 0; w < kWaves; ++w) {
                    const uint32_t c = s_cnt[b][w];
                    before += w < wv ? c : 0u;
                    tot += c;
                }
                if ((m[b] >> lane) & 1ull) {
                    l[b].group_id = -1;
                    out[base + before + (uint32_t)__popcll(m[b] & ((1ull << lane) - 1ull))] = l[b];
                }
                base += tot;
            }
            __syncthreads();
        }
    }
    __syncthreads();
    const uint32_t n = base;
    float mnx = INFINITY, mny = INFINITY, mxx = -INFINITY, mxy = -INFINITY;
    for (uint32_t i = threadIdx.x; i < n; i += kWG) {
        const LineSegment l = out[i];
        mnx = fminf(mnx, fminf(l.x1, l.x2));
        mny = fminf(mny, fminf(l.y1, l.y2));
        mxx = fmaxf(mxx, fmaxf(l.x1, l.x2));
        mxy = fmaxf(mxy, fmaxf(l.y1, l.y2));
    }
#pragma unroll
    for (int off = 32; off >= 1; off >>= 1) {
        mnx = fminf(mnx, __shfl_xor(mnx, off));
        mny = fminf(mny, __shfl_xor(mny, off));
        mxx = fmaxf(mxx, __shfl_xor(mxx, off));
        mxy = fmaxf(mxy, __shfl_xor(mxy, off));
    }
    if ((threadIdx.x & 63) == 0) {
        s_red[0][threadIdx.x >> 6] = mnx;
        s_red[1][threadIdx.x >> 6] = mny;
        s_red[2][threadIdx.x >> 6] = mxx;
        s_red[3][threadIdx.x >> 6] = mxy;
    }
    __syncthreads();
    if (threadIdx.x == 0) {
        for (int i = 1; i < kWaves; ++i) {
            mnx = fminf(mnx, s_red[0][i]);
            mny = fminf(mny, s_red[1][i]);
            mxx = fmaxf(mxx, s_red[2][i]);
            mxy = fmaxf(mxy, s_red[3][i]);
        }
        const float sx = mxx - mnx, sy = mxy - mny;
        gnorm[0] = mnx + 0.5f * sx;
        gnorm[1] = mny + 0.5f * sy;
        gnorm[2] = fmaxf(sx, sy);
        gctl[kGcLines] = n;
        gctl[kGcRemaining] = n;
        gctl[kGcRound] = 0u;
        gctl[kGcActive] = n;
        s_red[0][0] = gnorm[0];
        s_red[1][0] = gnorm[1];
        s_red[2][0] = gnorm[2];
    }
    if (with_model == 0u) return;
    __syncthreads();
    const float cx = s_red[0][0], cy = s_red[1][0], sc = s_red[2][0];
    for (uint32_t i = threadIdx.x; i < n; i += kWG) pencil_model_of(out[i], i, cx, cy, sc, all, round0);
}

__global__ __launch_bounds__(kWG) void lines_bbox_kernel(LineSegment* __restrict__ lines, uint32_t n,
                                                         uint32_t* __restrict__ gctl, float* __restrict__ gnorm) {
    __shared__ float s_red[4][kWaves];
    float mnx = INFINITY, mny = INFINITY, mxx = -INFINITY, mxy = -INFINITY;
    for (uint32_t i = threadIdx.x; i < n; i += kWG) {
        const LineSegment l = lines[i];
        mnx = fminf(mnx, fminf(l.x1, l.x2));
        mny = fminf(mny, fminf(l.y1, l.y2));
        mxx = fmaxf(mxx, fmaxf(l.x1, l.x2));
        mxy = fmaxf(mxy, fmaxf(l.y1, l.y2));
        lines[i].group_id = -1;
    }
#pragma unroll
    for (int off = 32; off >= 1; off >>= 1) {
        mnx = fminf(mnx, __shfl_xor(mnx, off));
        mny = fminf(mny, __shfl_xor(mny, off));
        mxx = fmaxf(mxx, __shfl_xor(mxx, off));
        mxy = fmaxf(mxy, __shfl_xor(mxy, off));
    }
    if ((threadIdx.x & 63) == 0) {
        s_red[0][threadIdx.x >> 6] = mnx;
        s_red[1][threadIdx.x >> 6] = mny;
        s_red[2][threadIdx.x >> 6] = mxx;
        s_red[3][threadIdx.x >> 6] = mxy;
    }
    __syncthreads();
    if (threadIdx.x == 0) {
        for (int i = 1; i < kWaves; ++i) {
            mnx = fminf(mnx, s_red[0][i]);
            mny = fminf(mny, s_red[1][i]);
            mxx = fmaxf(mxx, s_red[2][i]);
            mxy = fmaxf(mxy, s_red[3][i]);
        }
        const float sx = mxx - mnx, sy = mxy - mny;
        gnorm[0] = mnx + 0.5f * sx;
        gnorm[1] = mny + 0.5f * sy;
        gnorm[2] = fmaxf(sx, sy);
        gctl[kGcLines] = n;
        gctl[kGcRemaining] = n;
        gctl[kGcRound] = 0u;
        gctl[kGcActive] = n;
    }
}

__global__ __launch_bounds__(256) void pencil_model_kernel(const LineSegment* __restrict__ lines,
                                                           const uint32_t* __restrict__ gctl,
                                                           const float* __restrict__ gnorm, PencilTable all,
                                                           PencilTable round0) {
    const uint32_t i = blockIdx.x * 256 + threadIdx.x;
    if (i >= gctl[kGcLines]) return;
    pencil_model_of(lines[i], i, gnorm[0], gnorm[1], gnorm[2], all, round0);
}

__device__ __forceinline__ float pencil_error(float ax, float ay, float dx, float dy, float px, float py, float pz) {
    float vx, vy;
    if (fabsf(pz) < kEps) {
        vx = px;
        vy = py;
    } else {
        const float qx = px / pz, qy = py / pz;
        vx = qx - ax;
        vy = qy - ay;
    }
    const float nn = vx * vx + vy * vy;
    const float nrm = sqrtf(nn);
    const float ux = vx / nrm, uy = vy / nrm;
    return -fabsf(ux * dx + uy * dy) + 1.0f;
}

__device__ void smallest_eigenvector_3x3(const float c[9], float out[3]) {
    double A[3][3];
    double V[3][3] = {{1, 0, 0}, {0, 1, 0}, {0, 0, 1}};
    for (int i = 0; i < 3; ++i)
        for (int j = 0; j < 3; ++j) A[i][j] = 0.5 * ((double)c[i * 3 + j] + (double)c[j * 3 + i]);
    for (int sweep = 0; sweep < 64; ++sweep) {
        const double off = A[0][1] * A[0][1] + A[0][2] * A[0][2] + A[1][2] * A[1][2];
        const double dg = A[0][0] * A[0][0] + A[1][1] * A[1][1] + A[2][2] * A[2][2];
        if (off <= 1e-36 * dg) break;
        for (int p = 0; p < 2; ++p)
            for (int q = p + 1; q < 3; ++q) {
                if (A[p][q] == 0.0) continue;
                const double theta = (A[q][q] - A[p][p]) / (2.0 * A[p][q]);
                const double t = (theta >= 0 ? 1.0 : -1.0) / (fabs(theta) + sqrt(theta * theta + 1.0));
                const double cs = 1.0 / sqrt(t * t + 1.0), sn = t * cs;
                for (int k = 0; k < 3; ++k) {
                    const double akp = A[k][p], akq = A[k][q];
                    A[k][p] = cs * akp - sn * akq;
                    A[k][q] = sn * akp + cs * akq;
                }
                for (int k = 0; k < 3; ++k) {
                    const double apk = A[p][k], aqk = A[q][k];
                    A[p][k] = cs * apk - sn * aqk;
                    A[q][k] = sn * apk + cs * aqk;
                }
                for (int k = 0; k < 3; ++k) {
                    const double vkp = V[k][p], vkq = V[k][q];
                    V[k][p] = cs * vkp - sn * vkq;
                    V[k][q] = sn * vkp + cs * vkq;
                }
            }
    }
    int k = 0;
    if (A[1][1] < A[k][k]) k = 1;
    if (A[2][2] < A[k][k]) k = 2;
    const double nx = V[0][k], ny = V[1][k], nz = V[2][k];
    const double nn = sqrt(nx * nx + ny * ny + nz * nz);
    out[0] = (float)(nx / nn);
    out[1] = (float)(ny / nn);
    out[2] = (float)(nz / nn);
}

constexpr uint32_t kStage = 2048;
__device__ __forceinline__ void peel_body(const PencilTable& cur, const PencilTable& nxt, const PencilTable& all,
                                          unsigned long long* __restrict__ best_slots, uint64_t seed,
                                          float tol, float garbage_tol, int max_models,
                                          uint32_t* __restrict__ gctl, float4* __restrict__ stage_g,
                                          LineSegment* __restrict__ lines, float* __restrict__ models) {
    __shared__ uint32_t s_cnt[kWaves];
    __shared__ float s_bv[kWaves];
    __shared__ int s_bi[kWaves];
    __shared__ float s_h[3];
    __shared__ float4 s_stage[kStage];
    const int lane = threadIdx.x & 63, wv = threadIdx.x >> 6;
    const uint32_t n = gctl[kGcActive];
    const uint32_t round = gctl[kGcRound];
    if (gctl[kGcRemaining] < 2u || round >= (uint32_t)max_models) return;

#ifdef LR_PEEL_TIMING
    unsigned long long tm[6];
    tm[0] = wall_clock64();
#endif
    float r_ax = 0.f, r_ay = 0.f, r_dx = 0.f, r_dy = 0.f, r_len = 0.f, r_hx = 0.f, r_hy = 0.f, r_hz = 0.f;
    uint32_t r_orig = 0;
    if (threadIdx.x < n) {
        const uint32_t i = threadIdx.x;
        r_ax = cur.ax[i]; r_ay = cur.ay[i]; r_dx = cur.dx[i]; r_dy = cur.dy[i]; r_len = cur.len[i];
        r_hx = cur.hx[i]; r_hy = cur.hy[i]; r_hz = cur.hz[i]; r_orig = cur.orig[i];
    }

    if (threadIdx.x < 64) {
        unsigned long long key = threadIdx.x < (unsigned)kRansacBestSlots ? best_slots[threadIdx.x] : 0ull;
        if (threadIdx.x < (unsigned)kRansacBestSlots) best_slots[threadIdx.x] = 0ull;
#pragma unroll
        for (int off = 32; off >= 1; off >>= 1) {
            const unsigned long long o = ((unsigned long long)(uint32_t)__shfl_xor((int)(uint32_t)(key >> 32), off) << 32) |
                                         (uint32_t)__shfl_xor((int)(uint32_t)key, off);
            key = o > key ? o : key;
        }
        if (threadIdx.x == 0) {
            s_bv[0] = __uint_as_float((uint32_t)(key >> 32));
            s_bi[0] = key ? (int)(0xFFFFFFFFu - (uint32_t)key) : -1;
        }
    }
    __syncthreads();
    if (threadIdx.x == 0) {
        const int bi = s_bi[0];
        float hx = 0.f, hy = 0.f, hz = 0.f;
        if (bi >= 0) {
            uint32_t a, b;
            sample_pair(seed, round, (uint32_t)bi, n, a, b);
            const float ax = cur.hx[a], ay = cur.hy[a], az = cur.hz[a];
            const float bx = cur.hx[b], by = cur.hy[b], bz = cur.hz[b];
            hx = ay * bz - az * by;
            hy = az * bx - ax * bz;
            hz = ax * by - ay * bx;
        }
        s_h[0] = hx;
        s_h[1] = hy;
        s_h[2] = hz;
        if (round < (uint32_t)(kGcWords - kGcBestIter0)) gctl[kGcBestIter0 + round] = (uint32_t)bi;
    }
    __syncthreads();
    const float bx_ = s_h[0], by_ = s_h[1], bz_ = s_h[2];
#ifdef LR_PEEL_TIMING
    tm[1] = wall_clock64();
#endif

    uint32_t n_inl = 0;
    for (uint32_t i0 = 0; i0 < n; i0 += kWG) {
        const uint32_t i = i0 + threadIdx.x;
        bool in = false;
        float4 hl = make_float4(r_hx, r_hy, r_hz, r_len);
        if (i < n) {
            if (i0 == 0) {
                in = pencil_error(r_ax, r_ay, r_dx, r_dy, bx_, by_, bz_) < tol;
            } else {
                in = pencil_error(cur.ax[i], cur.ay[i], cur.dx[i], cur.dy[i], bx_, by_, bz_) < tol;
                if (in) hl = make_float4(cur.hx[i], cur.hy[i], cur.hz[i], cur.len[i]);
            }
        }
        uint32_t tot;
        const uint32_t r = block_rank(in, s_cnt, tot);
        if (in) {
            const uint32_t o = n_inl + r;
            if (o < kStage) s_stage[o] = hl;
            else stage_g[o] = hl;
        }
        n_inl += tot;
    }
    __syncthreads();

#ifdef LR_PEEL_TIMING
    tm[2] = wall_clock64();
#endif
    if (wv == 0) {
        const uint32_t m = n_inl ? n_inl : gctl[kGcLines];
        float acc[9];
#pragma unroll
        for (int k = 0; k < 9; ++k) acc[k] = 0.f;
        for (uint32_t j = lane; j < m; j += 64) {
            float4 hl;
            if (n_inl) hl = j < kStage ? s_stage[j] : stage_g[j];
            else hl = make_float4(all.hx[j], all.hy[j], all.hz[j], all.len[j]);
            const float hv[3] = {hl.x, hl.y, hl.z};
#pragma unroll
            for (int a = 0; a < 3; ++a) {
                const float t = hv[a] * hl.w;
#pragma unroll
                for (int b = 0; b < 3; ++b) acc[a * 3 + b] = acc[a * 3 + b] + t * hv[b];
            }
        }
#pragma unroll
        for (int k = 0; k < 9; ++k) acc[k] = wave_tree(acc[k]);
#ifdef LR_PEEL_TIMING
        tm[3] = wall_clock64();
#endif
        if (lane == 0) {
            float hf[3];
            smallest_eigenvector_3x3(acc, hf);
            s_h[0] = hf[0];
            s_h[1] = hf[1];
            s_h[2] = hf[2];
            if (round < (uint32_t)kMaxPeelModels) {
                models[round * 3 + 0] = hf[0];
                models[round * 3 + 1] = hf[1];
                models[round * 3 + 2] = hf[2];
            }
        }
    }
    __syncthreads();
    const float fx = s_h[0], fy = s_h[1], fz = s_h[2];
#ifdef LR_PEEL_TIMING
    tm[4] = wall_clock64();
#endif

    uint32_t n_next = 0, n_gone = 0;
    for (uint32_t i0 = 0; i0 < n; i0 += kWG) {
        const uint32_t i = i0 + threadIdx.x;
        bool stay = false, gone = false;
        if (i < n) {
            if (i0 != 0) {
                r_ax = cur.ax[i]; r_ay = cur.ay[i]; r_dx = cur.dx[i]; r_dy = cur.dy[i]; r_len = cur.len[i];
                r_hx = cur.hx[i]; r_hy = cur.hy[i]; r_hz = cur.hz[i]; r_orig = cur.orig[i];
            }
            const float e = pencil_error(r_ax, r_ay, r_dx, r_dy, fx, fy, fz);
            if (e < tol) {
                lines[r_orig].group_id = (int)round;
                gone = true;
            } else if (e >= tol && e < garbage_tol) {
                gone = true;
            } else {
                stay = true;
            }
        }
        uint32_t tot, tg;
        const uint32_t r = block_rank(stay, s_cnt, tot);
        if (stay) {
            const uint32_t o = n_next + r;
            nxt.ax[o] = r_ax; nxt.ay[o] = r_ay; nxt.dx[o] = r_dx; nxt.dy[o] = r_dy;
            nxt.len[o] = r_len; nxt.hx[o] = r_hx; nxt.hy[o] = r_hy; nxt.hz[o] = r_hz;
            nxt.orig[o] = r_orig;
        }
        (void)block_rank(gone, s_cnt, tg);
        n_next += tot;
        n_gone += tg;
    }
#ifdef LR_PEEL_TIMING
    if (threadIdx.x == 0) {
        tm[5] = wall_clock64();
        for (int q = 0; q < 5 && round < 4u; ++q) models[16 + round * 5 + q] = (float)(tm[q + 1] - tm[q]) * 0.01f;
    }
#endif
    if (threadIdx.x == 0) {
        gctl[kGcActive] = n_next;
        gctl[kGcRemaining] = gctl[kGcRemaining] - n_gone;
        gctl[kGcRound] = round + 1u;
    }
}

__global__ __launch_bounds__(kWG) void peel_kernel(PencilTable cur, PencilTable nxt, PencilTable all,
                                                   unsigned long long* __restrict__ best_slots, uint64_t seed,
                                                   float tol, float garbage_tol, int max_models,
                                                   uint32_t* __restrict__ gctl, float4* __restrict__ stage_g,
                                                   LineSegment* __restrict__ lines, float* __restrict__ models,
                                                   const uint32_t* __restrict__ counts, uint32_t cap_lines,
                                                   uint32_t* __restrict__ gather_dst) {
    peel_body(cur, nxt, all, best_slots, seed, tol, garbage_tol, max_models, gctl, stage_g, lines, models);
    if (gather_dst == nullptr) return;
    __syncthreads();
    const uint32_t t = threadIdx.x;
    const uint32_t* gw = gctl;
    if (t < 8) gather_dst[t] = counts[t];
    else if (t < 16) gather_dst[t] = gw[t - 8];
    else if (t < 56) gather_dst[t] = reinterpret_cast<const uint32_t*>(models)[t - 16];
    const uint32_t n = min(gw[kGcLines], cap_lines) * (uint32_t)(sizeof(LineSegment) / 4);
    const uint32_t* lw = reinterpret_cast<const uint32_t*>(lines);
    for (uint32_t i = t; i < n; i += kWG) gather_dst[64 + i] = lw[i];
}

}

int launch_filter_lines(const LineSegment* raw, const uint32_t* d_n_raw, uint32_t raw_cap, float min_length,
                        LineSegment* out, uint32_t* gctl, float* gnorm, const PencilTable* all, const PencilTable* round0,
                        hipStream_t s) {
    const bool with_model = all != nullptr && round0 != nullptr;
    hipLaunchKernelGGL(filter_lines_kernel, dim3(1), dim3(kWG), 0, s, raw, d_n_raw, raw_cap, min_length, out, gctl, gnorm,
                       with_model ? *all : PencilTable{}, with_model ? *round0 : PencilTable{}, with_model ? 1u : 0u);
    LR_HIP(hipGetLastError());
    return 0;
}

int launch_lines_bbox(LineSegment* lines, uint32_t n, uint32_t* gctl, float* gnorm, hipStream_t s) {
    hipLaunchKernelGGL(lines_bbox_kernel, dim3(1), dim3(kWG), 0, s, lines, n, gctl, gnorm);
    LR_HIP(hipGetLastError());
    return 0;
}

int launch_pencil_model(const LineSegment* lines, const uint32_t* gctl, const float* gnorm, PencilTable all,
                        PencilTable round0, uint32_t line_cap, hipStream_t s) {
    if (line_cap == 0) return 0;
    hipLaunchKernelGGL(pencil_model_kernel, dim3((line_cap + 255) / 256), dim3(256), 0, s, lines, gctl, gnorm, all, round0);
    LR_HIP(hipGetLastError());
    return 0;
}

int launch_peel(PencilTable cur, PencilTable nxt, PencilTable all, unsigned long long* best_slots, uint64_t seed,
                float tol, float garbage_tol, int max_models, uint32_t* gctl, float* stage4, LineSegment* lines,
                float* models, const uint32_t* counts, uint32_t cap_lines, void* gather_block, hipStream_t s) {
    hipLaunchKernelGGL(peel_kernel, dim3(1), dim3(kWG), 0, s, cur, nxt, all, best_slots, seed, tol, garbage_tol,
                       max_models, gctl, reinterpret_cast<float4*>(stage4), lines, models, counts, cap_lines,
                       static_cast<uint32_t*>(gather_block));
    LR_HIP(hipGetLastError());
    return 0;
}

}
```

librectify_amd/csrc/kernels_ransac.hip:

```cpp
#include <cstdlib>

#include "common.h"

namespace lramd {
namespace {

__device__ inline float wave_tree(float v) {
#pragma unroll
    for (int off = 32; off >= 1; off >>= 1) v = v + __shfl_xor(v, off);
    return v;
}

constexpr float kErrBand = 3e-6f;

__device__ __forceinline__ bool inlier_exact(float vx, float vy, float dx, float dy, float tol) {
    const float nn = vx * vx + vy * vy;
    const float nrm = sqrtf(nn);
    const float ux = vx / nrm, uy = vy / nrm;
    const float inc = fabsf(ux * dx + uy * dy);
    const float err = -inc + 1.0f;
    return err < tol;
}

__device__ __forceinline__ bool inlier_test(float vx, float vy, float dx, float dy, float tol) {
    const float nn = __builtin_fmaf(vx, vx, vy * vy);
    const float dot = __builtin_fmaf(vx, dx, vy * dy);
    const float e = 1.0f - fabsf(dot) * __builtin_amdgcn_rsqf(nn);
    bool in = e < tol - kErrBand;
    const bool sure = (in || e > tol + kErrBand) && nn > 1e-30f;
    if (__builtin_expect(!sure, 0)) in = inlier_exact(vx, vy, dx, dy, tol);
    return in;
}

struct Hyp {
    float cx, cy, sub;
    bool valid;
};
__device__ __forceinline__ Hyp make_hyp(const PencilSoA& m, uint32_t a, uint32_t b, float degeneracy_tol) {
    const float hax = m.hx[a], hay = m.hy[a], haz = m.hz[a];
    const float hbx = m.hx[b], hby = m.hy[b], hbz = m.hz[b];
    const float ex = hax - hbx, ey = hay - hby, ez = haz - hbz;
    const float dist = sqrtf((ex * ex + ey * ey) + ez * ez);
    Hyp h;
    h.valid = dist > degeneracy_tol;
    const float px = hay * hbz - haz * hby;
    const float py = haz * hbx - hax * hbz;
    const float pz = hax * hby - hay * hbx;
    const bool ideal = fabsf(pz) < kEps;
    h.cx = ideal ? px : px / pz;
    h.cy = ideal ? py : py / pz;
    h.sub = ideal ? 0.f : 1.f;
    return h;
}
__device__ __forceinline__ void hyp_v(const Hyp& h, float ax, float ay, float& vx, float& vy) {
    vx = h.sub != 0.f ? h.cx - ax : h.cx;
    vy = h.sub != 0.f ? h.cy - ay : h.cy;
}

constexpr float kTiny = 1e-30f;
struct EstConst {
    float k_in, k_out;
};
__device__ __forceinline__ EstConst est_const(float tol) {
    const float a = (1.0f - tol) + kErrBand, b = (1.0f - tol) - kErrBand;
    return EstConst{a * a, b * b};
}
typedef float f2 __attribute__((ext_vector_type(2)));
__device__ __forceinline__ void inlier_estimate2(const f2 cx, const f2 cy, const f2 nsub, float ax, float ay, float dx, float dy,
                                                 const EstConst& K, uint64_t& m_in0, uint64_t& m_un0, uint64_t& m_in1,
                                                 uint64_t& m_un1) {
    const f2 vx = __builtin_elementwise_fma(nsub, (f2){ax, ax}, cx), vy = __builtin_elementwise_fma(nsub, (f2){ay, ay}, cy);
    const f2 nn = __builtin_elementwise_fma(vx, vx, vy * vy);
    const f2 dot = __builtin_elementwise_fma(vx, (f2){dx, dx}, vy * (f2){dy, dy});
    const f2 dd = dot * dot;
    const f2 t_in = __builtin_elementwise_fma(nn, (f2){K.k_in, K.k_in}, (f2){kTiny, kTiny});
    const f2 t_out = __builtin_elementwise_fma(nn, (f2){K.k_out, K.k_out}, (f2){-kTiny, -kTiny});
    m_in0 = __builtin_amdgcn_fcmpf(dd.x, t_in.x, 2);
    m_in1 = __builtin_amdgcn_fcmpf(dd.y, t_in.y, 2);
    m_un0 = ~(m_in0 | __builtin_amdgcn_fcmpf(dd.x, t_out.x, 4));
    m_un1 = ~(m_in1 | __builtin_amdgcn_fcmpf(dd.y, t_out.y, 4));
}

constexpr int kScoreChunk = 512;
constexpr uint32_t kBestSlots = (uint32_t)kRansacBestSlots;
template <int kH>
__global__ __launch_bounds__(256) void ransac_score_kernel(PencilSoA m, uint32_t n_host, float tol, float degeneracy_tol,
                                                           uint32_t n_iter, uint64_t seed, uint32_t round_host,
                                                           const uint32_t* __restrict__ gctl, int max_models,
                                                           unsigned long long* __restrict__ best_slots) {
    __shared__ float s_tab[2][5][kScoreChunk];
    __shared__ unsigned long long s_key[4];
    const int lane = threadIdx.x & 63;
    const uint32_t hyp0 = (blockIdx.x * 4 + (threadIdx.x >> 6)) * kH;
    if (blockIdx.x * 4u * kH >= n_iter) return;
    uint32_t n = n_host, round = round_host;
    if (gctl) {
        n = gctl[kGcActive];
        round = gctl[kGcRound];
        if (gctl[kGcRemaining] < 2u || round >= (uint32_t)max_models) return;
    }
    float cx[kH], cy[kH], nsub[kH];
    bool valid[kH];
#pragma unroll
    for (int j = 0; j < kH; ++j) {
        uint32_t a, b;
        sample_pair(seed, round, min(hyp0 + (uint32_t)j, n_iter - 1u), n, a, b);
        const Hyp h = make_hyp(m, a, b, degeneracy_tol);
        cx[j] = h.cx;
        cy[j] = h.cy;
        nsub[j] = -h.sub;
        valid[j] = h.valid;
    }
    const EstConst K = est_const(tol);
    float acc[kH];
#pragma unroll
    for (int j = 0; j < kH; ++j) acc[j] = 0.f;
    auto stage = [&](int buf, uint32_t c0) {
        for (uint32_t t = threadIdx.x; t < (uint32_t)kScoreChunk; t += 256) {
            const uint32_t i = c0 + t;
            if (i < n) {
                s_tab[buf][0][t] = m.ax[i];
                s_tab[buf][1][t] = m.ay[i];
                s_tab[buf][2][t] = m.dx[i];
                s_tab[buf][3][t] = m.dy[i];
                s_tab[buf][4][t] = m.len[i];
            }
        }
    };
    stage(0, 0u);
    int buf = 0;
    for (uint32_t c0 = 0; c0 < n; c0 += kScoreChunk, buf ^= 1) {
        __syncthreads();
        if (c0 + kScoreChunk < n) stage(buf ^ 1, c0 + kScoreChunk);
        const uint32_t cn = min((uint32_t)kScoreChunk, n - c0);
        for (uint32_t t = lane; t < cn; t += 64) {
            const float ax = s_tab[buf][0][t], ay = s_tab[buf][1][t], dx = s_tab[buf][2][t], dy = s_tab[buf][3][t];
            const float len = s_tab[buf][4][t];
            uint64_t any_unsure = 0ull, mu[kH];
            static_assert(kH % 2 == 0, "hypotheses are scored in pairs");
#pragma unroll
            for (int j = 0; j < kH; j += 2) {
                uint64_t mi0, mi1;
                inlier_estimate2((f2){cx[j], cx[j + 1]}, (f2){cy[j], cy[j + 1]}, (f2){nsub[j], nsub[j + 1]}, ax, ay, dx, dy, K, mi0,
                                 mu[j], mi1, mu[j + 1]);
                acc[j] = acc[j] + (__builtin_amdgcn_inverse_ballot_w64(mi0 & ~mu[j]) ? len : 0.0f);
                acc[j + 1] = acc[j + 1] + (__builtin_amdgcn_inverse_ballot_w64(mi1 & ~mu[j + 1]) ? len : 0.0f);
                any_unsure |= mu[j] | mu[j + 1];
            }
            if (__builtin_expect(any_unsure != 0ull, 0)) {
#pragma unroll
                for (int j = 0; j < kH; ++j)
                    if (__builtin_amdgcn_inverse_ballot_w64(mu[j])) {
                        const float vx = __builtin_fmaf(nsub[j], ax, cx[j]), vy = __builtin_fmaf(nsub[j], ay, cy[j]);
                        acc[j] = acc[j] + (inlier_exact(vx, vy, dx, dy, tol) ? len : 0.0f);
                    }
            }
        }
    }
    unsigned long long key = 0ull;
#pragma unroll
    for (int j = 0; j < kH; ++j) {
        const float score = wave_tree(acc[j]);
        const uint32_t it = hyp0 + (uint32_t)j;
        if (valid[j] && it < n_iter && score > 0.0f) {
            const unsigned long long k = ((unsigned long long)__float_as_uint(score) << 32) | (unsigned long long)(0xFFFFFFFFu - it);
            key = k > key ? k : key;
        }
    }
    if (lane == 0) s_key[threadIdx.x >> 6] = key;
    __syncthreads();
    if (threadIdx.x != 0) return;
    for (int wv = 1; wv < 4; ++wv) key = s_key[wv] > key ? s_key[wv] : key;
    if (key != 0ull) (void)__hip_atomic_fetch_max(&best_slots[blockIdx.x % kBestSlots], key, __ATOMIC_RELAXED, __HIP_MEMORY_SCOPE_AGENT);
}

__global__ __launch_bounds__(64) void ransac_best_readout_kernel(unsigned long long* __restrict__ best_slots,
                                                                 uint32_t* __restrict__ host_best) {
    unsigned long long key = threadIdx.x < kBestSlots ? best_slots[threadIdx.x] : 0ull;
    if (threadIdx.x < kBestSlots) best_slots[threadIdx.x] = 0ull;
#pragma unroll
    for (int off = 32; off >= 1; off >>= 1) {
        const unsigned long long o = ((unsigned long long)(uint32_t)__shfl_xor((int)(uint32_t)(key >> 32), off) << 32) |
                                     (uint32_t)__shfl_xor((int)(uint32_t)key, off);
        key = o > key ? o : key;
    }
    if (threadIdx.x == 0) {
        host_best[0] = (uint32_t)(key >> 32);
        host_best[1] = key ? 0xFFFFFFFFu - (uint32_t)key : 0xFFFFFFFFu;
    }
}


template <int kH>
__global__ __launch_bounds__(256) void prosac_count_kernel(PencilSoA m, uint32_t n, float tol, float degeneracy_tol,
                                                           const uint32_t* __restrict__ sa,
                                                           const uint32_t* __restrict__ sb, uint32_t n_hyp,
                                                           uint32_t* __restrict__ counts) {
    __shared__ float s_tab[2][4][kScoreChunk];
    const int lane = threadIdx.x & 63;
    const uint32_t hyp0 = (blockIdx.x * 4 + (threadIdx.x >> 6)) * kH;
    if (blockIdx.x * 4u * kH >= n_hyp) return;
    float cx[kH], cy[kH], nsub[kH];
    bool valid[kH];
#pragma unroll
    for (int j = 0; j < kH; ++j) {
        const uint32_t h = min(hyp0 + (uint32_t)j, n_hyp - 1u);
        const Hyp hy = make_hyp(m, sa[h], sb[h], degeneracy_tol);
        cx[j] = hy.cx;
        cy[j] = hy.cy;
        nsub[j] = -hy.sub;
        valid[j] = hy.valid;
    }
    const EstConst K = est_const(tol);
    uint32_t cnt[kH];
#pragma unroll
    for (int j = 0; j < kH; ++j) cnt[j] = 0u;
    auto stage = [&](int buf, uint32_t c0) {
        for (uint32_t t = threadIdx.x; t < (uint32_t)kScoreChunk; t += 256) {
            const uint32_t i = c0 + t;
            if (i < n) {
                s_tab[buf][0][t] = m.ax[i];
                s_tab[buf][1][t] = m.ay[i];
                s_tab[buf][2][t] = m.dx[i];
                s_tab[buf][3][t] = m.dy[i];
            }
        }
    };
    stage(0, 0u);
    int buf = 0;
    for (uint32_t c0 = 0; c0 < n; c0 += kScoreChunk, buf ^= 1) {
        __syncthreads();
        if (c0 + kScoreChunk < n) stage(buf ^ 1, c0 + kScoreChunk);
        const uint32_t cn = min((uint32_t)kScoreChunk, n - c0);
        for (uint32_t t = lane; t < cn; t += 64) {
            const float ax = s_tab[buf][0][t], ay = s_tab[buf][1][t], dx = s_tab[buf][2][t], dy = s_tab[buf][3][t];
            uint64_t any_unsure = 0ull, mu[kH];
#pragma unroll
            for (int j = 0; j < kH; j += 2) {
                uint64_t mi0, mi1;
                inlier_estimate2((f2){cx[j], cx[j + 1]}, (f2){cy[j], cy[j + 1]}, (f2){nsub[j], nsub[j + 1]}, ax, ay, dx, dy, K, mi0,
                                 mu[j], mi1, mu[j + 1]);
                cnt[j] += __builtin_amdgcn_inverse_ballot_w64(mi0 & ~mu[j]) ? 1u : 0u;
                cnt[j + 1] += __builtin_amdgcn_inverse_ballot_w64(mi1 & ~mu[j + 1]) ? 1u : 0u;
                any_unsure |= mu[j] | mu[j + 1];
            }
            if (__builtin_expect(any_unsure != 0ull, 0)) {
#pragma unroll
                for (int j = 0; j < kH; ++j)
                    if (__builtin_amdgcn_inverse_ballot_w64(mu[j])) {
                        const float vx = __builtin_fmaf(nsub[j], ax, cx[j]), vy = __builtin_fmaf(nsub[j], ay, cy[j]);
                        cnt[j] += inlier_exact(vx, vy, dx, dy, tol) ? 1u : 0u;
                    }
            }
        }
    }
#pragma unroll
    for (int j = 0; j < kH; ++j) {
        uint32_t c = cnt[j];
#pragma unroll
        for (int off = 32; off >= 1; off >>= 1) c += (uint32_t)__shfl_xor((int)c, off);
        if (lane == 0 && hyp0 + (uint32_t)j < n_hyp) counts[hyp0 + j] = valid[j] ? c : 0xFFFFFFFFu;
    }
}

__global__ __launch_bounds__(256) void prosac_flags_kernel(PencilSoA m, uint32_t n, float px, float py, float pz, float tol,
                                                           uint8_t* __restrict__ flags) {
    const uint32_t i = blockIdx.x * 256 + threadIdx.x;
    if (i >= n) return;
    float vx, vy;
    if (fabsf(pz) < kEps) {
        vx = px;
        vy = py;
    } else {
        vx = px / pz - m.ax[i];
        vy = py / pz - m.ay[i];
    }
    flags[i] = inlier_exact(vx, vy, m.dx[i], m.dy[i], tol) ? 1 : 0;
}

__global__ __launch_bounds__(1024) void prosac_records_kernel(const uint32_t* __restrict__ counts, uint32_t n_hyp, uint32_t best_in,
                                                              uint32_t* __restrict__ rec ,
                                                              uint32_t cap) {
    __shared__ uint32_t s_max[1024];
    __shared__ uint32_t s_cnt[1024];
    const uint32_t L = (n_hyp + 1023u) / 1024u;
    const uint32_t i0 = threadIdx.x * L, i1 = min(n_hyp, i0 + L);
    uint32_t mx = 0;
    for (uint32_t i = i0; i < i1; ++i) {
        const uint32_t c = counts[i];
        if (c != 0xFFFFFFFFu) mx = max(mx, c);
    }
    s_max[threadIdx.x] = mx;
    __syncthreads();
    for (int off = 1; off < 1024; off <<= 1) {
        const uint32_t o = threadIdx.x >= (unsigned)off ? s_max[threadIdx.x - off] : 0u;
        __syncthreads();
        s_max[threadIdx.x] = max(s_max[threadIdx.x], o);
        __syncthreads();
    }
    uint32_t run = max(best_in, threadIdx.x ? s_max[threadIdx.x - 1] : 0u);
    uint32_t n = 0;
    for (uint32_t i = i0; i < i1; ++i) {
        const uint32_t c = counts[i];
        if (c != 0xFFFFFFFFu && c > run) {
            run = c;
            ++n;
        }
    }
    s_cnt[threadIdx.x] = n;
    __syncthreads();
    for (int off = 1; off < 1024; off <<= 1) {
        const uint32_t o = threadIdx.x >= (unsigned)off ? s_cnt[threadIdx.x - off] : 0u;
        __syncthreads();
        s_cnt[threadIdx.x] += o;
        __syncthreads();
    }
    uint32_t pos = s_cnt[threadIdx.x] - n;
    run = max(best_in, threadIdx.x ? s_max[threadIdx.x - 1] : 0u);
    for (uint32_t i = i0; i < i1; ++i) {
        const uint32_t c = counts[i];
        if (c != 0xFFFFFFFFu && c > run) {
            run = c;
            if (pos < cap) rec[1 + pos] = i;
            ++pos;
        }
    }
    if (threadIdx.x == 1023) rec[0] = s_cnt[1023];
}

__global__ __launch_bounds__(256) void prosac_record_flags_kernel(PencilSoA m, uint32_t n, const uint32_t* __restrict__ sa,
                                                                  const uint32_t* __restrict__ sb,
                                                                  const uint32_t* __restrict__ rec, uint32_t cap, float tol,
                                                                  uint8_t* __restrict__ flags) {
    const uint32_t r = blockIdx.y;
    if (r >= min(rec[0], cap)) return;
    const uint32_t i = blockIdx.x * 256 + threadIdx.x;
    if (i >= n) return;
    const uint32_t j = rec[1 + r];
    const uint32_t a = sa[j], b = sb[j];
    const float hax = m.hx[a], hay = m.hy[a], haz = m.hz[a];
    const float hbx = m.hx[b], hby = m.hy[b], hbz = m.hz[b];
    const float px = hay * hbz - haz * hby;
    const float py = haz * hbx - hax * hbz;
    const float pz = hax * hby - hay * hbx;
    float vx, vy;
    if (fabsf(pz) < kEps) {
        vx = px;
        vy = py;
    } else {
        vx = px / pz - m.ax[i];
        vy = py / pz - m.ay[i];
    }
    flags[(size_t)r * n + i] = inlier_exact(vx, vy, m.dx[i], m.dy[i], tol) ? 1 : 0;
}

constexpr int kHtMax = 65;
__global__ __launch_bounds__(1024) void ht_votes_kernel(PencilSoA m, const int32_t* __restrict__ pa,
                                                        const int32_t* __restrict__ pb, int n_pairs, int ht,
                                                        float* __restrict__ peak ) {
    __shared__ unsigned long long acc[kHtMax * kHtMax];
    __shared__ unsigned long long s_best[16];
    __shared__ int s_pos[16];
    const float k = floorf(ht / 2.f), k1 = k - 1;
    for (int i = threadIdx.x; i < ht * ht; i += 1024) acc[i] = 0ull;
    __syncthreads();
    for (int i = threadIdx.x; i < n_pairs; i += 1024) {
        const int a = pa[i], b = pb[i];
        float x = m.hy[a] * m.hz[b] - m.hz[a] * m.hy[b];
        float y = m.hz[a] * m.hx[b] - m.hx[a] * m.hz[b];
        float z = m.hx[a] * m.hy[b] - m.hy[a] * m.hx[b];
        if (fabsf(x) < 0.0001f && fabsf(y) < 0.0001f && fabsf(z) < 0.0001f) continue;
        const float zz = (x * x + y * y) + z * z;
        if (zz > 0.0f) {
            const float nn = sqrtf(zz);
            x = x / nn;
            y = y / nn;
            z = z / nn;
        }
        if (z < 0.f) {
            x = -x;
            y = -y;
        }
        const int u = (int)roundf(k1 * x + k);
        const int v = (int)roundf(k1 * y + k);
        const float vote = m.len[a] + m.len[b];
        atomicAdd(&acc[u * ht + v], (unsigned long long)(vote * 1048576.0f + 0.5f));
    }
    __syncthreads();
    unsigned long long bv = 0ull;
    int bp = 0x7FFFFFFF;
    for (int i = threadIdx.x; i < ht * ht; i += 1024) {
        const int u = i / ht, v = i - u * ht;
        const int pos = v * ht + u;
        const unsigned long long val = acc[i];
        if (val > bv || (val == bv && pos < bp)) {
            bv = val;
            bp = pos;
        }
    }
#pragma unroll
    for (int off = 32; off >= 1; off >>= 1) {
        const unsigned long long ov = __shfl_xor(bv, off);
        const int op = __shfl_xor(bp, off);
        if (ov > bv || (ov == bv && op < bp)) {
            bv = ov;
            bp = op;
        }
    }
    if ((threadIdx.x & 63) == 0) {
        s_best[threadIdx.x >> 6] = bv;
        s_pos[threadIdx.x >> 6] = bp;
    }
    __syncthreads();
    if (threadIdx.x == 0) {
        for (int w = 1; w < 16; ++w)
            if (s_best[w] > bv || (s_best[w] == bv && s_pos[w] < bp)) {
                bv = s_best[w];
                bp = s_pos[w];
            }
        const int max_v = bp / ht, max_u = bp - max_v * ht;
        float p0 = (max_u - k) / k1, p1 = (max_v - k) / k1;
        const float pn = sqrtf((p0 * p0 + p1 * p1) + 0.f * 0.f);
        if (pn > 1.f) {
            p0 = p0 / pn;
            p1 = p1 / pn;
        }
        peak[0] = p0;
        peak[1] = p1;
        peak[2] = sqrtf(1.f - (p0 * p0 + p1 * p1));
    }
}

__global__ __launch_bounds__(256) void ht_weights_kernel(PencilSoA m, uint32_t n, const float* __restrict__ peak,
                                                         float* __restrict__ weights) {
    const uint32_t i = blockIdx.x * 256 + threadIdx.x;
    if (i >= n) return;
    const float px = peak[0], py = peak[1], pz = peak[2];
    float vx, vy;
    if (fabsf(pz) < kEps) {
        vx = px;
        vy = py;
    } else {
        vx = px / pz - m.ax[i];
        vy = py / pz - m.ay[i];
    }
    const float nrm = sqrtf(vx * vx + vy * vy);
    const float ux = vx / nrm, uy = vy / nrm;
    const float inc = fabsf(ux * m.dx[i] + uy * m.dy[i]);
    const float i2 = inc * inc;
    weights[i] = i2 * i2;
}

struct RefineSeg {
    float x1, y1, x2, y2, dx, dy, len;
};

__global__ __launch_bounds__(256) void refine_pairs_kernel(const RefineSeg* __restrict__ seg, uint32_t n,
                                                           uint2* __restrict__ edges, uint32_t* __restrict__ n_edges,
                                                           uint32_t cap) {
    __shared__ RefineSeg si[64], sj[64];
    const uint32_t bi = blockIdx.y, bj = blockIdx.x;
    if (bj < bi) return;
    const uint32_t i0 = bi * 64, j0 = bj * 64;
    for (uint32_t t = threadIdx.x; t < 128; t += 256) {
        const uint32_t idx = (t < 64) ? i0 + t : j0 + (t - 64);
        RefineSeg v{0, 0, 0, 0, 0, 0, 1};
        if (idx < n) v = seg[idx];
        if (t < 64) si[t] = v; else sj[t - 64] = v;
    }
    __syncthreads();
    for (uint32_t p = threadIdx.x; p < 64 * 64; p += 256) {
        const uint32_t a = p >> 6, b = p & 63;
        const uint32_t i = i0 + a, j = j0 + b;
        if (i >= n || j >= n || j <= i) continue;
        const RefineSeg A = si[a], B = sj[b];
        if (fabsf(A.dx * B.dx + A.dy * B.dy) < 0.99) continue;
        const bool i_short = A.len < B.len;
        const RefineSeg R = i_short ? B : A;
        const RefineSeg O = i_short ? A : B;
        const float nx = -R.dy, ny = R.dx;
        const float ax = O.x1 - R.x1, ay = O.y1 - R.y1, bx = O.x2 - R.x1, by = O.y2 - R.y1;
        const float w00 = (ax * R.dx + ay * R.dy) / R.len, w01 = (ax * nx + ay * ny) / R.len;
        const float w10 = (bx * R.dx + by * R.dy) / R.len, w11 = (bx * nx + by * ny) / R.len;
        if (fmaxf(fabsf(w01), fabsf(w11)) < 0.02) {
            const bool any_gt = (w00 > -0.5) || (w10 > -0.5);
            const bool any_lt = (w00 < 1.5) || (w10 < 1.5);
            if (any_gt && any_lt) {
                const uint32_t slot = atomicAdd(n_edges, 1u);
                if (slot < cap) edges[slot] = make_uint2(i, j);
            }
        }
    }
}

__device__ inline float sgn1(float x) { return x >= 0.f ? 1.f : -1.f; }
constexpr int kChtMax = 128;
constexpr int kChtLinesPerBlock = 512;

template <bool kSub>
__global__ __launch_bounds__(256) void cht_votes_kernel(PencilSoA m, const uint32_t* __restrict__ idx, uint32_t n, int d,
                                                        unsigned long long* __restrict__ acc,
                                                        unsigned long long* __restrict__ n_votes) {
    extern __shared__ uint32_t s_acc[];
    for (int i = threadIdx.x; i < d * d; i += 256) s_acc[i] = 0u;
    __syncthreads();
    const float sc = (float)(d - 1);
    const int lane = threadIdx.x & 63, wv = threadIdx.x >> 6;
    const uint32_t lo = blockIdx.x * kChtLinesPerBlock;
    const uint32_t hi = min(n, lo + kChtLinesPerBlock);
    uint32_t cast = 0;
    for (uint32_t li = lo + wv; li < hi; li += 4) {
        const uint32_t i = idx ? idx[li] : li;
        const float a = m.hx[i], b = m.hy[i], c = m.hz[i];
        const float al = sgn1(a * b), be = sgn1(b * c), ga = sgn1(a * c);
        const float d1 = c + ga * a, d2 = c + be * b, d3 = a + al * b;
        float px[4], py[4];
        bool ok[4];
        ok[0] = ok[3] = d1 != 0.f;
        ok[1] = d2 != 0.f;
        ok[2] = d3 != 0.f;
        px[0] = al * a / d1;   py[0] = -al * c / d1;
        px[1] = b / d2;        py[1] = 0.f;
        px[2] = 0.f;           py[2] = b / d3;
        px[3] = -al * a / d1;  py[3] = al * c / d1;
        const uint32_t vote = (uint32_t)(m.len[i] * 65536.0f + 0.5f);
#pragma unroll
        for (int s = 0; s < 3; ++s) {
            if (!ok[s] || !ok[s + 1]) continue;
            const float x0 = roundf((px[s] + 1.f) * 0.5f * sc), y0 = roundf((py[s] + 1.f) * 0.5f * sc);
            const float x1 = roundf((px[s + 1] + 1.f) * 0.5f * sc), y1 = roundf((py[s + 1] + 1.f) * 0.5f * sc);
            if (!(x0 >= 0.f && x0 <= sc && y0 >= 0.f && y0 <= sc && x1 >= 0.f && x1 <= sc && y1 >= 0.f && y1 <= sc)) continue;
            const int steps = (int)roundf(fmaxf(fabsf(x1 - x0), fabsf(y1 - y0))) + 1;
            const float sx = steps > 1 ? (x1 - x0) / (float)(steps - 1) : 0.f;
            const float sy = steps > 1 ? (y1 - y0) / (float)(steps - 1) : 0.f;
            for (int j = lane; j < steps; j += 64) {
                const int xi = (int)roundf(x0 + (float)j * sx), yi = (int)roundf(y0 + (float)j * sy);
                atomicAdd(&s_acc[yi * d + xi], vote);
            }
            cast += (uint32_t)steps;
        }
    }
    __syncthreads();
    for (int i = threadIdx.x; i < d * d; i += 256) {
        const uint32_t v = s_acc[i];
        if (v) atomicAdd(&acc[i], kSub ? (unsigned long long)0 - (unsigned long long)v : (unsigned long long)v);
    }
    if (n_votes && lane == 0 && cast) atomicAdd(n_votes, (unsigned long long)cast);
}

__global__ __launch_bounds__(1024) void cht_peak_kernel(const unsigned long long* __restrict__ acc, uint32_t cells,
                                                        uint32_t* __restrict__ out) {
    __shared__ unsigned long long s_v[16];
    __shared__ uint32_t s_i[16];
    unsigned long long bv = 0ull;
    uint32_t bi = 0xFFFFFFFFu;
    for (uint32_t i = threadIdx.x; i < cells; i += 1024) {
        const unsigned long long v = acc[i];
        if (bi == 0xFFFFFFFFu || v > bv) {
            bv = v;
            bi = i;
        }
    }
#pragma unroll
    for (int off = 32; off >= 1; off >>= 1) {
        const uint32_t olo = (uint32_t)__shfl_xor((int)(uint32_t)bv, off), ohi = (uint32_t)__shfl_xor((int)(uint32_t)(bv >> 32), off);
        const unsigned long long ov = ((unsigned long long)ohi << 32) | olo;
        const uint32_t oi = (uint32_t)__shfl_xor((int)bi, off);
        if (oi != 0xFFFFFFFFu && (bi == 0xFFFFFFFFu || ov > bv || (ov == bv && oi < bi))) {
            bv = ov;
            bi = oi;
        }
    }
    if ((threadIdx.x & 63) == 0) {
        s_v[threadIdx.x >> 6] = bv;
        s_i[threadIdx.x >> 6] = bi;
    }
    __syncthreads();
    if (threadIdx.x == 0) {
        for (int k = 1; k < 16; ++k) {
            const unsigned long long ov = s_v[k];
            const uint32_t oi = s_i[k];
            if (oi != 0xFFFFFFFFu && (bi == 0xFFFFFFFFu || ov > bv || (ov == bv && oi < bi))) {
                bv = ov;
                bi = oi;
            }
        }
        out[0] = bi == 0xFFFFFFFFu ? 0u : bi;
        out[1] = (uint32_t)bv;
        out[2] = (uint32_t)(bv >> 32);
    }
}

}

static int cht_check_size(int d) {
    if (d < 8 || d > kChtMax) {
        set_error("diamond-space accumulator: size must be in [8, 128]");
        return 1;
    }
    return 0;
}

int launch_cht_accumulate(PencilSoA m, uint32_t n, int d, unsigned long long* acc, hipStream_t s) {
    if (cht_check_size(d)) return 1;
    LR_HIP(hipMemsetAsync(acc, 0, (size_t)d * d * sizeof(unsigned long long), s));
    return launch_cht_votes(m, nullptr, n, d, acc, false, nullptr, s);
}

int launch_cht_votes(PencilSoA m, const uint32_t* idx, uint32_t n, int d, unsigned long long* acc, bool subtract,
                     unsigned long long* n_votes, hipStream_t s) {
    if (cht_check_size(d)) return 1;
    if (n == 0) return 0;
    const uint32_t blocks = (n + kChtLinesPerBlock - 1) / kChtLinesPerBlock;
    const size_t lds = (size_t)d * d * sizeof(uint32_t);
    if (subtract) hipLaunchKernelGGL(cht_votes_kernel<true>, dim3(blocks), dim3(256), lds, s, m, idx, n, d, acc, n_votes);
    else hipLaunchKernelGGL(cht_votes_kernel<false>, dim3(blocks), dim3(256), lds, s, m, idx, n, d, acc, n_votes);
    LR_HIP(hipGetLastError());
    return 0;
}

int launch_cht_peak(const unsigned long long* acc, int d, uint32_t* out3, hipStream_t s) {
    hipLaunchKernelGGL(cht_peak_kernel, dim3(1), dim3(1024), 0, s, acc, (uint32_t)(d * d), out3);
    LR_HIP(hipGetLastError());
    return 0;
}

int launch_refine_pairs(const void* seg, uint32_t n, void* edges, uint32_t* n_edges, uint32_t cap, hipStream_t s) {
    const uint32_t nb = (n + 63) / 64;
    hipLaunchKernelGGL(refine_pairs_kernel, dim3(nb, nb), dim3(256), 0, s, (const RefineSeg*)seg, n, (uint2*)edges,
                       n_edges, cap);
    LR_HIP(hipGetLastError());
    return 0;
}

int launch_prosac_count(PencilSoA m, uint32_t n, float tol, float degeneracy_tol, const uint32_t* sa,
                        const uint32_t* sb, uint32_t n_hyp, uint32_t* counts, hipStream_t s) {
    if (n_hyp == 0) return 0;
    if (n_hyp >= 16384u) {
        hipLaunchKernelGGL(prosac_count_kernel<8>, dim3((n_hyp + 31) / 32), dim3(256), 0, s, m, n, tol, degeneracy_tol, sa,
                           sb, n_hyp, counts);
    } else {
        hipLaunchKernelGGL(prosac_count_kernel<2>, dim3((n_hyp + 7) / 8), dim3(256), 0, s, m, n, tol, degeneracy_tol, sa, sb,
                           n_hyp, counts);
    }
    LR_HIP(hipGetLastError());
    return 0;
}

int launch_prosac_records(PencilSoA m, uint32_t n, const uint32_t* sa, const uint32_t* sb, const uint32_t* counts,
                          uint32_t n_hyp, uint32_t best_in, float tol, uint32_t* rec, uint32_t cap, uint8_t* flags, hipStream_t s) {
    if (n_hyp == 0 || n == 0) return 0;
    hipLaunchKernelGGL(prosac_records_kernel, dim3(1), dim3(1024), 0, s, counts, n_hyp, best_in, rec, cap);
    hipLaunchKernelGGL(prosac_record_flags_kernel, dim3((n + 255) / 256, cap), dim3(256), 0, s, m, n, sa, sb, rec, cap, tol, flags);
    LR_HIP(hipGetLastError());
    return 0;
}

int launch_prosac_flags(PencilSoA m, uint32_t n, float px, float py, float pz, float tol, uint8_t* flags, hipStream_t s) {
    if (n == 0) return 0;
    hipLaunchKernelGGL(prosac_flags_kernel, dim3((n + 255) / 256), dim3(256), 0, s, m, n, px, py, pz, tol, flags);
    LR_HIP(hipGetLastError());
    return 0;
}

int launch_ht_weights(PencilSoA m, uint32_t n, const int32_t* pa, const int32_t* pb, int n_pairs, int ht, float* peak,
                      float* weights, hipStream_t s) {
    if (ht > kHtMax || ht < 3) {
        set_error("launch_ht_weights: accumulator size out of range");
        return 1;
    }
    hipLaunchKernelGGL(ht_votes_kernel, dim3(1), dim3(1024), 0, s, m, pa, pb, n_pairs, ht, peak);
    hipLaunchKernelGGL(ht_weights_kernel, dim3((n + 255) / 256), dim3(256), 0, s, m, n, peak, weights);
    LR_HIP(hipGetLastError());
    return 0;
}

static void launch_score(PencilSoA m, uint32_t n, float tol, float degeneracy_tol, uint32_t n_iter, uint64_t seed,
                         uint32_t round, const uint32_t* gctl, int max_models, unsigned long long* best_slots, hipStream_t s) {
    if (n_iter >= 65536u) {
        hipLaunchKernelGGL(ransac_score_kernel<8>, dim3((n_iter + 31) / 32), dim3(256), 0, s, m, n, tol, degeneracy_tol,
                           n_iter, seed, round, gctl, max_models, best_slots);
    } else {
        hipLaunchKernelGGL(ransac_score_kernel<4>, dim3((n_iter + 15) / 16), dim3(256), 0, s, m, n, tol, degeneracy_tol,
                           n_iter, seed, round, gctl, max_models, best_slots);
    }
}

int launch_ransac_score(PencilSoA m, uint32_t n, float tol, float degeneracy_tol, uint32_t n_iter, uint64_t seed,
                        uint32_t round, unsigned long long* best_slots, uint32_t* host_best, hipStream_t s) {
    if (n < 2 || n_iter == 0) {
        set_error("launch_ransac_score: need at least 2 lines and 1 iteration");
        return 1;
    }
    launch_score(m, n, tol, degeneracy_tol, n_iter, seed, round, nullptr, 0, best_slots, s);
    hipLaunchKernelGGL(ransac_best_readout_kernel, dim3(1), dim3(64), 0, s, best_slots, host_best);
    LR_HIP(hipGetLastError());
    return 0;
}

int launch_ransac_score_dev(PencilSoA m, const uint32_t* gctl, int max_models, float tol, float degeneracy_tol,
                            uint32_t n_iter, uint64_t seed, unsigned long long* best_slots, hipStream_t s) {
    if (n_iter == 0) return 0;
    launch_score(m, 0u, tol, degeneracy_tol, n_iter, seed, 0u, gctl, max_models, best_slots, s);
    LR_HIP(hipGetLastError());
    return 0;
}


}
```

Measured before the change: 10370.

## Split head-frame page-locking, skip ready waits, fuse RANSAC score with peel

The first few frames of a batch are now page-locked in pieces by several register threads at once, and each piece is uploaded as soon as it is ready, so the first transfers start sooner. Lanes query the upload event and skip hipStreamWaitEvent when the transfer has already completed. The flood JIT sleep is disabled once all uploads are enqueued. Per-model RANSAC scoring and peeling are fused into one score_peel launch using a ticket word, which removes one kernel launch per model. The change adds complexity, more registrations and unregistrations, and new diagnostic timing.

Measured after the change: 10230. 1.4% lower.

```diff
diff --git a/librectify_amd/csrc/batch.hip b/librectify_amd/csrc/batch.hip
--- a/librectify_amd/csrc/batch.hip
+++ b/librectify_amd/csrc/batch.hip
@@ -12,6 +12,7 @@
                              LineSegment* out, int capacity, int* n_lines, const RectificationConfig* cfg,
                              ImageTransform* transforms) {
     if (batch <= 0) return 0;
+    const double t_entry = now_ms();
     const uint8_t* d_images = static_cast<const uint8_t*>(d_images_);
     const uint8_t* const* h_frames = reinterpret_cast<const uint8_t* const*>(h_frames_);
     const size_t bpp = (size_t)pix_bytes(format);
@@ -84,7 +85,9 @@
     };
     static const bool batch_stats = std::getenv("LIBRECTIFY_BATCH_STATS") != nullptr;
     std::atomic<long long> up_wait_us{0}, lane_wait_us{0}, lead_sum_us{0};
-    std::atomic<int> late_frames{0};
+    std::atomic<int> late_frames{0}, waits_skipped{0};
+    std::atomic<long long> first_up_us{-1}, first_kernel_us{-1}, last_up_done_us{-1};
+    std::atomic<int> uploads_enqueued{h_frames ? 0 : 1};
     static const int register_threads = std::getenv("LIBRECTIFY_REGISTER_FRAMES") ? std::max(0, std::atoi(std::getenv("LIBRECTIFY_REGISTER_FRAMES"))) : 4;
     if (c->register_slow_calls > 0) --c->register_slow_calls;
     const bool reg_frames = register_threads > 0 && h_frames != nullptr && any_pageable && stride >= w && c->register_slow_calls == 0;
@@ -119,6 +122,30 @@
     std::atomic<int> reg_slow{0};
     std::vector<std::atomic<int>> reg_ready(reg_frames ? (size_t)batch : 0);
     for (auto& a : reg_ready) a.store(0, std::memory_order_relaxed);
+#ifndef LR_HEAD_FRAMES
+#define LR_HEAD_FRAMES 4
+#endif
+    constexpr int kHeadFrames = LR_HEAD_FRAMES;
+    struct HeadPiece {
+        uintptr_t lo = 0, hi = 0;
+        std::atomic<int> state{0};
+        double ms = 0.0, t_done = 0.0;
+    };
+    const int n_head = reg_frames && register_threads > 1 && pitch == row_bytes ? register_threads : 0;
+    const int n_head_frames = n_head ? std::min(kHeadFrames, batch) : 0;
+    std::vector<HeadPiece> head((size_t)n_head * (size_t)n_head_frames);
+    for (int i = 0; i < n_head_frames; ++i) {
+        const RegPlan& p = plan[(size_t)i];
+        if (p.hi <= p.lo) continue;
+        constexpr uintptr_t kPage = 4096;
+        const uintptr_t pages = (p.hi - p.lo) / kPage, per = (pages + (uintptr_t)n_head - 1) / (uintptr_t)n_head;
+        for (int k = 0; k < n_head; ++k) {
+            head[(size_t)(i * n_head + k)].lo = std::min(p.hi, p.lo + (uintptr_t)k * per * kPage);
+            head[(size_t)(i * n_head + k)].hi = std::min(p.hi, p.lo + (uintptr_t)(k + 1) * per * kPage);
+        }
+        reg_ready[(size_t)i].store(3, std::memory_order_relaxed);
+    }
+    std::atomic<int> head_next{0};
     std::atomic<int> reg_next{0};
     std::vector<std::thread> reg_pool;
     if (reg_frames)
@@ -126,6 +153,19 @@
             reg_pool.emplace_back([&]() {
                 (void)hipSetDevice(c->device);
                 bind_this_thread_near(c->device);
+                for (int k = head_next.fetch_add(1, std::memory_order_relaxed); k < (int)head.size(); k = head_next.fetch_add(1, std::memory_order_relaxed)) {
+                    HeadPiece& hp = head[(size_t)k];
+                    int ok = 2;
+                    const double t_r0 = now_ms();
+                    if (hp.hi <= hp.lo) ok = 1;
+                    else if (!abort_all.load(std::memory_order_relaxed))
+                        ok = hipHostRegister(reinterpret_cast<void*>(hp.lo), hp.hi - hp.lo, hipHostRegisterDefault) == hipSuccess ? 1 : 2;
+                    if (ok == 2) (void)hipGetLastError();
+                    hp.t_done = now_ms();
+                    hp.ms = hp.t_done - t_r0;
+                    if (ok == 1 && hp.hi > hp.lo && hp.ms * 6.0e6 > (double)(hp.hi - hp.lo)) reg_slow.fetch_add(1, std::memory_order_relaxed);
+                    hp.state.store(ok, std::memory_order_release);
+                }
                 for (int i = reg_next.fetch_add(1, std::memory_order_relaxed); i < batch && !abort_all.load(std::memory_order_relaxed);
                      i = reg_next.fetch_add(1, std::memory_order_relaxed)) {
                     if (reg_slow.load(std::memory_order_relaxed) >= 2) break;
@@ -162,20 +202,54 @@
             if (batch_stats) up_wait_us.fetch_add((long long)((now_ms() - t_w0) * 1e3));
             if (abort_all.load(std::memory_order_relaxed)) return;
             slot_busy[(size_t)slot].store(1, std::memory_order_relaxed);
-            if (reg_frames) {
+            const bool in_pieces = i < n_head_frames && plan[(size_t)i].hi > plan[(size_t)i].lo;
+            if (reg_frames && !in_pieces) {
                 int sp2 = 0;
                 int expect = 0;
                 if (!reg_ready[(size_t)i].compare_exchange_strong(expect, 2, std::memory_order_acq_rel))
                     while (reg_ready[(size_t)i].load(std::memory_order_acquire) == 3 && !abort_all.load(std::memory_order_relaxed)) nap(sp2);
             }
-            const bool registered = reg_frames && reg_ready[(size_t)i].load(std::memory_order_acquire) == 1;
+            const bool registered = reg_frames && !in_pieces && reg_ready[(size_t)i].load(std::memory_order_acquire) == 1;
             uint8_t* stage = locked[(size_t)i] ? nullptr : reinterpret_cast<uint8_t*>(c->ring.stage[(size_t)slot].get());
             uint8_t* dimg = reinterpret_cast<uint8_t*>(c->ring.img[(size_t)slot].get());
             const double t_u0 = now_ms();
             Event e_dbg;
             if (lane_debug && e_dbg.create() == hipSuccess) (void)hipEventRecord(e_dbg, c->copy_stream);
             int up_rc = 0;
-            if (registered) {
+            bool sent = false;
+            if (in_pieces) {
+                const RegPlan& p = plan[(size_t)i];
+                const uint8_t* f = h_frames[i];
+                for (int r = 0; r < p.r_lo; ++r) std::memcpy(stage + (size_t)r * row_bytes, f + (size_t)r * pitch, row_bytes);
+                for (int r = p.r_hi; r < h; ++r) std::memcpy(stage + (size_t)r * row_bytes, f + (size_t)r * pitch, row_bytes);
+                const uintptr_t b0 = reinterpret_cast<uintptr_t>(f) + (size_t)p.r_lo * row_bytes, b1 = reinterpret_cast<uintptr_t>(f) + (size_t)p.r_hi * row_bytes;
+                sent = true;
+                for (int k = 0; k < n_head && sent; ++k) {
+                    HeadPiece& hp = head[(size_t)(i * n_head + k)];
+                    int sp2 = 0, st;
+                    while ((st = hp.state.load(std::memory_order_acquire)) != 1 && st != 2 && !abort_all.load(std::memory_order_relaxed)) nap(sp2);
+                    if (st != 1) {
+                        sent = false;
+                        break;
+                    }
+                    const uintptr_t lo = std::max(hp.lo, b0), hi = std::min(hp.hi, b1);
+                    if (hi <= lo) continue;
+                    if (hipMemcpyAsync(dimg + (lo - reinterpret_cast<uintptr_t>(f)), reinterpret_cast<const void*>(lo), hi - lo, hipMemcpyHostToDevice, c->copy_stream) != hipSuccess) {
+                        (void)hipGetLastError();
+                        set_error("upload: transfer of a registered frame failed");
+                        up_rc = 1;
+                        break;
+                    }
+                    if (batch_stats && first_up_us.load() < 0) first_up_us.store((long long)((now_ms() - t_entry) * 1e3));
+                }
+                if (abort_all.load(std::memory_order_relaxed)) return;
+                if (sent) {
+                    slot_edges[(size_t)slot].r_lo = p.r_lo;
+                    slot_edges[(size_t)slot].r_hi = p.r_hi;
+                }
+            }
+            if (sent || up_rc) {
+            } else if (registered) {
                 const RegPlan& p = plan[(size_t)i];
                 const uint8_t* f = h_frames[i];
                 for (int r = 0; r < p.r_lo; ++r) std::memcpy(stage + (size_t)r * row_bytes, f + (size_t)r * pitch, row_bytes);
@@ -203,6 +277,12 @@
                 return;
             }
             enq[(size_t)i].store(slot + 1, std::memory_order_release);
+            if (batch_stats && first_up_us.load() < 0) first_up_us.store((long long)((now_ms() - t_entry) * 1e3));
+            if (i == batch - 1) {
+                uploads_enqueued.store(1, std::memory_order_release);
+                if (batch_stats && hipEventSynchronize(c->ring_ev[(size_t)slot]) == hipSuccess)
+                    last_up_done_us.store((long long)((now_ms() - t_entry) * 1e3));
+            }
             if (lane_debug) {
                 const double t_u1 = now_ms();
                 float dma = 0.f;
@@ -237,9 +317,23 @@
                 while ((slot = enq[(size_t)b].load(std::memory_order_acquire) - 1) < 0 && !abort_all.load(std::memory_order_relaxed)) nap(spins);
                 if (batch_stats) lane_wait_us.fetch_add((long long)((now_ms() - t_w0) * 1e3));
                 if (slot < 0) return;
-                if (hipStreamWaitEvent(l->stream, c->ring_ev[(size_t)slot], 0) != hipSuccess) {
-                    set_error("hipStreamWaitEvent failed");
-                    return fail();
+#ifdef LR_CMP_ALWAYS_WAIT
+                const hipError_t up_done = hipErrorNotReady;
+#else
+                const hipError_t up_done = hipEventQuery(c->ring_ev[(size_t)slot]);
+#endif
+                if (up_done == hipSuccess) {
+                    if (batch_stats) waits_skipped.fetch_add(1);
+                } else {
+                    (void)hipGetLastError();
+                    if (up_done != hipErrorNotReady) {
+                        set_error("hipEventQuery of a frame's transfer failed");
+                        return fail();
+                    }
+                    if (hipStreamWaitEvent(l->stream, c->ring_ev[(size_t)slot], 0) != hipSuccess) {
+                        set_error("hipStreamWaitEvent failed");
+                        return fail();
+                    }
                 }
                 img = c->ring.img[(size_t)slot].get();
                 img_stride = w;
@@ -260,8 +354,12 @@
             } else {
                 img = d_images + (size_t)b * image_stride * bpp;
             }
+#ifndef LR_CMP_NO_DRAIN_SPIN
+            if (S > 1 && h_frames) l->flood_jit_sleep_us = uploads_enqueued.load(std::memory_order_acquire) ? 0 : 20;
+#endif
             std::vector<LineSegment> res;
             const double t_f0 = now_ms();
+            if (batch_stats && first_kernel_us.load() < 0) first_kernel_us.store((long long)((t_f0 - t_entry) * 1e3));
             if (ctx_find_groups_device(l, img, format, w, h, img_stride, min_length, refine, res)) return fail();
             if (batch_stats && h_frames && l->opt.timing_on) {
                 float lead = 0.f;
@@ -304,10 +402,24 @@
     if (h_frames) (void)hipStreamSynchronize(c->copy_stream);
     for (auto& t : reg_pool) t.join();
     if (reg_slow.load() >= 2) c->register_slow_calls = 32;
-    if (reg_frames)
+    const double t_rel0 = now_ms();
+    if (reg_frames) {
+        for (HeadPiece& hp : head)
+            if (hp.hi > hp.lo && hp.state.load(std::memory_order_acquire) == 1 && hipHostUnregister(reinterpret_cast<void*>(hp.lo)) != hipSuccess) (void)hipGetLastError();
         for (int i = 0; i < batch; ++i)
             if (reg_ready[(size_t)i].load(std::memory_order_acquire) == 1 && hipHostUnregister(reinterpret_cast<void*>(plan[(size_t)i].lo)) != hipSuccess)
                 (void)hipGetLastError();
+    }
+    if (batch_stats && h_frames) {
+        const double t_ret = now_ms();
+        std::fprintf(stderr, "   from the call's entry: first transfer enqueued at %.3f ms, first frame handed to its lane at %.3f ms; the last transfer was over %.3f ms before the call returned; %d of %d frames needed no device-side wait for their transfer; releasing the frames took %.3f ms\n",
+                     first_up_us.load() * 1e-3, first_kernel_us.load() * 1e-3, last_up_done_us.load() < 0 ? -1.0 : t_ret - t_entry - last_up_done_us.load() * 1e-3,
+                     waits_skipped.load(), batch, t_ret - t_rel0);
+        for (size_t k = 0; k < head.size(); ++k)
+            if (head[k].hi > head[k].lo)
+                std::fprintf(stderr, "   frame %d, piece %d: %.2f MB page-locked in %.3f ms, ready %.3f ms after the call's entry\n", (int)k / n_head, (int)k % n_head,
+                             (double)(head[k].hi - head[k].lo) * 1e-6, head[k].ms, head[k].t_done - t_entry);
+    }
     for (lr_context* l : lanes) l->sleep_in_wait = false;
     c->flood_logbig_off = false;
     c->flood_log_min = c->flood_log_walk = 0;
diff --git a/librectify_amd/csrc/common.h b/librectify_amd/csrc/common.h
--- a/librectify_amd/csrc/common.h
+++ b/librectify_amd/csrc/common.h
@@ -205,6 +205,7 @@
     const float* hz;
 };
 constexpr int kRansacBestSlots = 32;
+constexpr int kRansacTicketWord = kRansacBestSlots;
 int launch_ransac_score(PencilSoA m, uint32_t n, float tol, float degeneracy_tol, uint32_t n_iter, uint64_t seed,
                         uint32_t round, unsigned long long* best_slots, uint32_t* host_best, hipStream_t s);
 int launch_ransac_score_dev(PencilSoA m, const uint32_t* gctl, int max_models, float tol, float degeneracy_tol,
@@ -241,6 +242,10 @@
                 LineSegment* lines, float* models,
                 const uint32_t* counts, uint32_t cap_lines, void* gather_block ,
                 hipStream_t s);
+int launch_score_peel(PencilTable cur, PencilTable nxt, PencilTable all, unsigned long long* best_slots , uint64_t seed,
+                      float tol, float degeneracy_tol, float garbage_tol, uint32_t n_iter, int max_models, uint32_t* gctl,
+                      float* stage4, LineSegment* lines, float* models, const uint32_t* counts, uint32_t cap_lines,
+                      void* gather_block, hipStream_t s);
 int launch_cht_accumulate(PencilSoA m, uint32_t n, int d, unsigned long long* acc, hipStream_t s);
 int launch_cht_votes(PencilSoA m, const uint32_t* idx, uint32_t n, int d, unsigned long long* acc, bool subtract,
                      unsigned long long* n_votes, hipStream_t s);
diff --git a/librectify_amd/csrc/context.hip b/librectify_amd/csrc/context.hip
--- a/librectify_amd/csrc/context.hip
+++ b/librectify_amd/csrc/context.hip
@@ -223,12 +223,12 @@
         check(c->d_gctl.alloc(kGcWords), "hipMalloc(peeling control block)");
         check(c->d_gnorm.alloc(4), "hipMalloc(normalisation)");
         check(c->d_models.alloc(64), "hipMalloc(models)");
-        check(c->d_best_slots.alloc(kRansacBestSlots), "hipMalloc(best slots)");
+        check(c->d_best_slots.alloc(kRansacBestSlots + 1), "hipMalloc(best slots)");
         check(c->h_counts.alloc(128), "hipHostMalloc(counts)");
         check(c->h_best.alloc(2), "hipHostMalloc(best)");
         if (bad == hipSuccess) check(hipMemset(c->d_models, 0, 64 * sizeof(float)), "hipMemset(models)");
         if (bad == hipSuccess) check(hipMemset(c->d_counts, 0, 64 * sizeof(uint32_t)), "hipMemset(counts)");
-        if (bad == hipSuccess) check(hipMemset(c->d_best_slots, 0, kRansacBestSlots * sizeof(unsigned long long)), "hipMemset(best slots)");
+        if (bad == hipSuccess) check(hipMemset(c->d_best_slots, 0, (kRansacBestSlots + 1) * sizeof(unsigned long long)), "hipMemset(best slots)");
         if (bad != hipSuccess) {
             (void)hipGetLastError();
             const std::string msg = std::string("lr_context_create: ") + what + " failed: " + hipGetErrorString(bad);
diff --git a/librectify_amd/csrc/frame.hip b/librectify_amd/csrc/frame.hip
--- a/librectify_amd/csrc/frame.hip
+++ b/librectify_amd/csrc/frame.hip
@@ -253,11 +253,20 @@
     if (!model_done && launch_pencil_model(c->d_flines, c->d_gctl, c->d_gnorm, all, tab[0], line_cap, c->stream)) return 1;
     const float degeneracy_tol = 0.05f;
     for (int k = 0; k < max_models; ++k) {
+        const bool last = gather && k == max_models - 1;
+#ifndef LR_CMP_NO_FUSED_ROUND
+        if (n_iter > 0) {
+            if (launch_score_peel(tab[k & 1], tab[(k + 1) & 1], all, c->d_best_slots, seed, tol, degeneracy_tol, garbage_tol,
+                                  (uint32_t)n_iter, max_models, c->d_gctl, c->d_inl, c->d_flines, c->d_models, c->d_counts,
+                                  (uint32_t)std::min<size_t>(c->res_lines_cap, c->d_flines.cap()), last ? c->h_res.get() : nullptr, c->stream))
+                return 1;
+            continue;
+        }
+#endif
         if (n_iter > 0 &&
             launch_ransac_score_dev(tab[k & 1].soa(), c->d_gctl, max_models, tol, degeneracy_tol, (uint32_t)n_iter, seed,
                                     c->d_best_slots, c->stream))
             return 1;
-        const bool last = gather && k == max_models - 1;
         if (launch_peel(tab[k & 1], tab[(k + 1) & 1], all, c->d_best_slots, seed, tol, garbage_tol,
                         max_models, c->d_gctl, c->d_inl, c->d_flines, c->d_models, c->d_counts,
                         (uint32_t)std::min<size_t>(c->res_lines_cap, c->d_flines.cap()), last ? c->h_res.get() : nullptr, c->stream))
diff --git a/librectify_amd/csrc/kernels_groups.hip b/librectify_amd/csrc/kernels_groups.hip
--- a/librectify_amd/csrc/kernels_groups.hip
+++ b/librectify_amd/csrc/kernels_groups.hip
@@ -1,16 +1,11 @@
 #include "common.h"
+#include "ransac_score.h"
 
 namespace lramd {
 namespace {
 
 constexpr int kWG = 1024;
 constexpr int kWaves = kWG / 64;
-
-__device__ __forceinline__ float wave_tree(float v) {
-#pragma unroll
-    for (int off = 32; off >= 1; off >>= 1) v = v + __shfl_xor(v, off);
-    return v;
-}
 
 __device__ __forceinline__ uint32_t block_rank(bool flag, uint32_t* s_cnt, uint32_t& total) {
     const int lane = threadIdx.x & 63, wv = threadIdx.x >> 6;
@@ -264,12 +259,12 @@
                                           unsigned long long* __restrict__ best_slots, uint64_t seed,
                                           float tol, float garbage_tol, int max_models,
                                           uint32_t* __restrict__ gctl, float4* __restrict__ stage_g,
-                                          LineSegment* __restrict__ lines, float* __restrict__ models) {
+                                          LineSegment* __restrict__ lines, float* __restrict__ models,
+                                          float4* __restrict__ s_stage ) {
     __shared__ uint32_t s_cnt[kWaves];
     __shared__ float s_bv[kWaves];
     __shared__ int s_bi[kWaves];
     __shared__ float s_h[3];
-    __shared__ float4 s_stage[kStage];
     const int lane = threadIdx.x & 63, wv = threadIdx.x >> 6;
     const uint32_t n = gctl[kGcActive];
     const uint32_t round = gctl[kGcRound];
@@ -437,6 +432,18 @@
     }
 }
 
+__device__ __forceinline__ void gather_results(const uint32_t* __restrict__ gw, const float* __restrict__ models,
+                                               const LineSegment* __restrict__ lines, const uint32_t* __restrict__ counts,
+                                               uint32_t cap_lines, uint32_t* __restrict__ gather_dst) {
+    const uint32_t t = threadIdx.x;
+    if (t < 8) gather_dst[t] = counts[t];
+    else if (t < 16) gather_dst[t] = gw[t - 8];
+    else if (t < 56) gather_dst[t] = reinterpret_cast<const uint32_t*>(models)[t - 16];
+    const uint32_t n = min(gw[kGcLines], cap_lines) * (uint32_t)(sizeof(LineSegment) / 4);
+    const uint32_t* lw = reinterpret_cast<const uint32_t*>(lines);
+    for (uint32_t i = t; i < n; i += kWG) gather_dst[64 + i] = lw[i];
+}
+
 __global__ __launch_bounds__(kWG) void peel_kernel(PencilTable cur, PencilTable nxt, PencilTable all,
                                                    unsigned long long* __restrict__ best_slots, uint64_t seed,
                                                    float tol, float garbage_tol, int max_models,
@@ -444,17 +451,45 @@
                                                    LineSegment* __restrict__ lines, float* __restrict__ models,
                                                    const uint32_t* __restrict__ counts, uint32_t cap_lines,
                                                    uint32_t* __restrict__ gather_dst) {
-    peel_body(cur, nxt, all, best_slots, seed, tol, garbage_tol, max_models, gctl, stage_g, lines, models);
+    __shared__ float4 s_stage[kStage];
+    peel_body(cur, nxt, all, best_slots, seed, tol, garbage_tol, max_models, gctl, stage_g, lines, models, s_stage);
     if (gather_dst == nullptr) return;
     __syncthreads();
-    const uint32_t t = threadIdx.x;
-    const uint32_t* gw = gctl;
-    if (t < 8) gather_dst[t] = counts[t];
-    else if (t < 16) gather_dst[t] = gw[t - 8];
-    else if (t < 56) gather_dst[t] = reinterpret_cast<const uint32_t*>(models)[t - 16];
-    const uint32_t n = min(gw[kGcLines], cap_lines) * (uint32_t)(sizeof(LineSegment) / 4);
-    const uint32_t* lw = reinterpret_cast<const uint32_t*>(lines);
-    for (uint32_t i = t; i < n; i += kWG) gather_dst[64 + i] = lw[i];
+    gather_results(gctl, models, lines, counts, cap_lines, gather_dst);
+}
+
+template <int kH>
+__global__ __launch_bounds__(kWG) void score_peel_kernel(PencilTable cur, PencilTable nxt, PencilTable all,
+                                                         unsigned long long* __restrict__ best_slots, uint64_t seed,
+                                                         float tol, float degeneracy_tol, float garbage_tol, uint32_t n_iter,
+                                                         int max_models, uint32_t* __restrict__ gctl,
+                                                         float4* __restrict__ stage_g, LineSegment* __restrict__ lines,
+                                                         float* __restrict__ models, const uint32_t* __restrict__ counts,
+                                                         uint32_t cap_lines, uint32_t* __restrict__ gather_dst) {
+    static_assert(sizeof(float4) * kStage >= sizeof(float) * kScoreTabFloats, "the scoring's table chunks fit the peel's stage");
+    __shared__ float4 s_lds[kStage];
+    __shared__ unsigned long long s_key[kWaves];
+    __shared__ uint32_t s_last;
+    const uint32_t n = gctl[kGcActive], round = gctl[kGcRound];
+    if (gctl[kGcRemaining] < 2u || round >= (uint32_t)max_models) {
+        if (gather_dst != nullptr && blockIdx.x == 0) gather_results(gctl, models, lines, counts, cap_lines, gather_dst);
+        return;
+    }
+    const unsigned long long key = score_block<kH, kWG>(PencilSoA{cur.ax, cur.ay, cur.dx, cur.dy, cur.len, cur.hx, cur.hy, cur.hz}, n, round, tol, degeneracy_tol, n_iter, seed,
+                                                       reinterpret_cast<float*>(s_lds), s_key);
+    uint32_t* ticket = reinterpret_cast<uint32_t*>(best_slots + kRansacTicketWord);
+    if (threadIdx.x == 0) {
+        if (key != 0ull) (void)__hip_atomic_fetch_max(&best_slots[blockIdx.x % (uint32_t)kRansacBestSlots], key, __ATOMIC_RELAXED, __HIP_MEMORY_SCOPE_AGENT);
+        s_last = __hip_atomic_fetch_add(ticket, 1u, __ATOMIC_RELEASE, __HIP_MEMORY_SCOPE_AGENT) == gridDim.x - 1u ? 1u : 0u;
+    }
+    __syncthreads();
+    if (s_last == 0u) return;
+    __builtin_amdgcn_fence(__ATOMIC_ACQUIRE, "agent");
+    if (threadIdx.x == 0) *ticket = 0u;
+    peel_body(cur, nxt, all, best_slots, seed, tol, garbage_tol, max_models, gctl, stage_g, lines, models, s_lds);
+    if (gather_dst == nullptr) return;
+    __syncthreads();
+    gather_results(gctl, models, lines, counts, cap_lines, gather_dst);
 }
 
 }
@@ -493,4 +528,21 @@
     return 0;
 }
 
-}
+int launch_score_peel(PencilTable cur, PencilTable nxt, PencilTable all, unsigned long long* best_slots, uint64_t seed,
+                      float tol, float degeneracy_tol, float garbage_tol, uint32_t n_iter, int max_models, uint32_t* gctl,
+                      float* stage4, LineSegment* lines, float* models, const uint32_t* counts, uint32_t cap_lines,
+                      void* gather_block, hipStream_t s) {
+    if (n_iter >= 65536u) {
+        hipLaunchKernelGGL(score_peel_kernel<8>, dim3((n_iter + kWaves * 8 - 1) / (kWaves * 8)), dim3(kWG), 0, s, cur, nxt, all,
+                           best_slots, seed, tol, degeneracy_tol, garbage_tol, n_iter, max_models, gctl,
+                           reinterpret_cast<float4*>(stage4), lines, models, counts, cap_lines, static_cast<uint32_t*>(gather_block));
+    } else {
+        hipLaunchKernelGGL(score_peel_kernel<4>, dim3((n_iter + kWaves * 4 - 1) / (kWaves * 4)), dim3(kWG), 0, s, cur, nxt, all,
+                           best_slots, seed, tol, degeneracy_tol, garbage_tol, n_iter, max_models, gctl,
+                           reinterpret_cast<float4*>(stage4), lines, models, counts, cap_lines, static_cast<uint32_t*>(gather_block));
+    }
+    LR_HIP(hipGetLastError());
+    return 0;
+}
+
+}
diff --git a/librectify_amd/csrc/kernels_ransac.hip b/librectify_amd/csrc/kernels_ransac.hip
--- a/librectify_amd/csrc/kernels_ransac.hip
+++ b/librectify_amd/csrc/kernels_ransac.hip
@@ -1,97 +1,19 @@
 #include <cstdlib>
 
 #include "common.h"
+#include "ransac_score.h"
 
 namespace lramd {
 namespace {
 
-__device__ inline float wave_tree(float v) {
-#pragma unroll
-    for (int off = 32; off >= 1; off >>= 1) v = v + __shfl_xor(v, off);
-    return v;
-}
-
-constexpr float kErrBand = 3e-6f;
-
-__device__ __forceinline__ bool inlier_exact(float vx, float vy, float dx, float dy, float tol) {
-    const float nn = vx * vx + vy * vy;
-    const float nrm = sqrtf(nn);
-    const float ux = vx / nrm, uy = vy / nrm;
-    const float inc = fabsf(ux * dx + uy * dy);
-    const float err = -inc + 1.0f;
-    return err < tol;
-}
-
-__device__ __forceinline__ bool inlier_test(float vx, float vy, float dx, float dy, float tol) {
-    const float nn = __builtin_fmaf(vx, vx, vy * vy);
-    const float dot = __builtin_fmaf(vx, dx, vy * dy);
-    const float e = 1.0f - fabsf(dot) * __builtin_amdgcn_rsqf(nn);
-    bool in = e < tol - kErrBand;
-    const bool sure = (in || e > tol + kErrBand) && nn > 1e-30f;
-    if (__builtin_expect(!sure, 0)) in = inlier_exact(vx, vy, dx, dy, tol);
-    return in;
-}
-
-struct Hyp {
-    float cx, cy, sub;
-    bool valid;
-};
-__device__ __forceinline__ Hyp make_hyp(const PencilSoA& m, uint32_t a, uint32_t b, float degeneracy_tol) {
-    const float hax = m.hx[a], hay = m.hy[a], haz = m.hz[a];
-    const float hbx = m.hx[b], hby = m.hy[b], hbz = m.hz[b];
-    const float ex = hax - hbx, ey = hay - hby, ez = haz - hbz;
-    const float dist = sqrtf((ex * ex + ey * ey) + ez * ez);
-    Hyp h;
-    h.valid = dist > degeneracy_tol;
-    const float px = hay * hbz - haz * hby;
-    const float py = haz * hbx - hax * hbz;
-    const float pz = hax * hby - hay * hbx;
-    const bool ideal = fabsf(pz) < kEps;
-    h.cx = ideal ? px : px / pz;
-    h.cy = ideal ? py : py / pz;
-    h.sub = ideal ? 0.f : 1.f;
-    return h;
-}
-__device__ __forceinline__ void hyp_v(const Hyp& h, float ax, float ay, float& vx, float& vy) {
-    vx = h.sub != 0.f ? h.cx - ax : h.cx;
-    vy = h.sub != 0.f ? h.cy - ay : h.cy;
-}
-
-constexpr float kTiny = 1e-30f;
-struct EstConst {
-    float k_in, k_out;
-};
-__device__ __forceinline__ EstConst est_const(float tol) {
-    const float a = (1.0f - tol) + kErrBand, b = (1.0f - tol) - kErrBand;
-    return EstConst{a * a, b * b};
-}
-typedef float f2 __attribute__((ext_vector_type(2)));
-__device__ __forceinline__ void inlier_estimate2(const f2 cx, const f2 cy, const f2 nsub, float ax, float ay, float dx, float dy,
-                                                 const EstConst& K, uint64_t& m_in0, uint64_t& m_un0, uint64_t& m_in1,
-                                                 uint64_t& m_un1) {
-    const f2 vx = __builtin_elementwise_fma(nsub, (f2){ax, ax}, cx), vy = __builtin_elementwise_fma(nsub, (f2){ay, ay}, cy);
-    const f2 nn = __builtin_elementwise_fma(vx, vx, vy * vy);
-    const f2 dot = __builtin_elementwise_fma(vx, (f2){dx, dx}, vy * (f2){dy, dy});
-    const f2 dd = dot * dot;
-    const f2 t_in = __builtin_elementwise_fma(nn, (f2){K.k_in, K.k_in}, (f2){kTiny, kTiny});
-    const f2 t_out = __builtin_elementwise_fma(nn, (f2){K.k_out, K.k_out}, (f2){-kTiny, -kTiny});
-    m_in0 = __builtin_amdgcn_fcmpf(dd.x, t_in.x, 2);
-    m_in1 = __builtin_amdgcn_fcmpf(dd.y, t_in.y, 2);
-    m_un0 = ~(m_in0 | __builtin_amdgcn_fcmpf(dd.x, t_out.x, 4));
-    m_un1 = ~(m_in1 | __builtin_amdgcn_fcmpf(dd.y, t_out.y, 4));
-}
-
-constexpr int kScoreChunk = 512;
 constexpr uint32_t kBestSlots = (uint32_t)kRansacBestSlots;
 template <int kH>
 __global__ __launch_bounds__(256) void ransac_score_kernel(PencilSoA m, uint32_t n_host, float tol, float degeneracy_tol,
                                                            uint32_t n_iter, uint64_t seed, uint32_t round_host,
                                                            const uint32_t* __restrict__ gctl, int max_models,
                                                            unsigned long long* __restrict__ best_slots) {
-    __shared__ float s_tab[2][5][kScoreChunk];
+    __shared__ float s_tab[kScoreTabFloats];
     __shared__ unsigned long long s_key[4];
-    const int lane = threadIdx.x & 63;
-    const uint32_t hyp0 = (blockIdx.x * 4 + (threadIdx.x >> 6)) * kH;
     if (blockIdx.x * 4u * kH >= n_iter) return;
     uint32_t n = n_host, round = round_host;
     if (gctl) {
@@ -99,78 +21,8 @@
         round = gctl[kGcRound];
         if (gctl[kGcRemaining] < 2u || round >= (uint32_t)max_models) return;
     }
-    float cx[kH], cy[kH], nsub[kH];
-    bool valid[kH];
-#pragma unroll
-    for (int j = 0; j < kH; ++j) {
-        uint32_t a, b;
-        sample_pair(seed, round, min(hyp0 + (uint32_t)j, n_iter - 1u), n, a, b);
-        const Hyp h = make_hyp(m, a, b, degeneracy_tol);
-        cx[j] = h.cx;
-        cy[j] = h.cy;
-        nsub[j] = -h.sub;
-        valid[j] = h.valid;
-    }
-    const EstConst K = est_const(tol);
-    float acc[kH];
-#pragma unroll
-    for (int j = 0; j < kH; ++j) acc[j] = 0.f;
-    auto stage = [&](int buf, uint32_t c0) {
-        for (uint32_t t = threadIdx.x; t < (uint32_t)kScoreChunk; t += 256) {
-            const uint32_t i = c0 + t;
-            if (i < n) {
-                s_tab[buf][0][t] = m.ax[i];
-                s_tab[buf][1][t] = m.ay[i];
-                s_tab[buf][2][t] = m.dx[i];
-                s_tab[buf][3][t] = m.dy[i];
-                s_tab[buf][4][t] = m.len[i];
-            }
-        }
-    };
-    stage(0, 0u);
-    int buf = 0;
-    for (uint32_t c0 = 0; c0 < n; c0 += kScoreChunk, buf ^= 1) {
-        __syncthreads();
-        if (c0 + kScoreChunk < n) stage(buf ^ 1, c0 + kScoreChunk);
-        const uint32_t cn = min((uint32_t)kScoreChunk, n - c0);
-        for (uint32_t t = lane; t < cn; t += 64) {
-            const float ax = s_tab[buf][0][t], ay = s_tab[buf][1][t], dx = s_tab[buf][2][t], dy = s_tab[buf][3][t];
-            const float len = s_tab[buf][4][t];
-            uint64_t any_unsure = 0ull, mu[kH];
-            static_assert(kH % 2 == 0, "hypotheses are scored in pairs");
-#pragma unroll
-            for (int j = 0; j < kH; j += 2) {
-                uint64_t mi0, mi1;
-                inlier_estimate2((f2){cx[j], cx[j + 1]}, (f2){cy[j], cy[j + 1]}, (f2){nsub[j], nsub[j + 1]}, ax, ay, dx, dy, K, mi0,
-                                 mu[j], mi1, mu[j + 1]);
-                acc[j] = acc[j] + (__builtin_amdgcn_inverse_ballot_w64(mi0 & ~mu[j]) ? len : 0.0f);
-                acc[j + 1] = acc[j + 1] + (__builtin_amdgcn_inverse_ballot_w64(mi1 & ~mu[j + 1]) ? len : 0.0f);
-                any_unsure |= mu[j] | mu[j + 1];
-            }
-            if (__builtin_expect(any_unsure != 0ull, 0)) {
-#pragma unroll
-                for (int j = 0; j < kH; ++j)
-                    if (__builtin_amdgcn_inverse_ballot_w64(mu[j])) {
-                        const float vx = __builtin_fmaf(nsub[j], ax, cx[j]), vy = __builtin_fmaf(nsub[j], ay, cy[j]);
-                        acc[j] = acc[j] + (inlier_exact(vx, vy, dx, dy, tol) ? len : 0.0f);
-                    }
-            }
-        }
-    }
-    unsigned long long key = 0ull;
-#pragma unroll
-    for (int j = 0; j < kH; ++j) {
-        const float score = wave_tree(acc[j]);
-        const uint32_t it = hyp0 + (uint32_t)j;
-        if (valid[j] && it < n_iter && score > 0.0f) {
-            const unsigned long long k = ((unsigned long long)__float_as_uint(score) << 32) | (unsigned long long)(0xFFFFFFFFu - it);
-            key = k > key ? k : key;
-        }
-    }
-    if (lane == 0) s_key[threadIdx.x >> 6] = key;
-    __syncthreads();
+    const unsigned long long key = score_block<kH, 256>(m, n, round, tol, degeneracy_tol, n_iter, seed, s_tab, s_key);
     if (threadIdx.x != 0) return;
-    for (int wv = 1; wv < 4; ++wv) key = s_key[wv] > key ? s_key[wv] : key;
     if (key != 0ull) (void)__hip_atomic_fetch_max(&best_slots[blockIdx.x % kBestSlots], key, __ATOMIC_RELAXED, __HIP_MEMORY_SCOPE_AGENT);
 }
 
diff --git a/librectify_amd/csrc/ransac_score.h b/librectify_amd/csrc/ransac_score.h
--- /dev/null
+++ b/librectify_amd/csrc/ransac_score.h
@@ -0,0 +1,169 @@
+#pragma once
+#include "common.h"
+
+namespace lramd {
+namespace {
+
+__device__ __forceinline__ float wave_tree(float v) {
+#pragma unroll
+    for (int off = 32; off >= 1; off >>= 1) v = v + __shfl_xor(v, off);
+    return v;
+}
+
+constexpr float kErrBand = 3e-6f;
+
+__device__ __forceinline__ bool inlier_exact(float vx, float vy, float dx, float dy, float tol) {
+    const float nn = vx * vx + vy * vy;
+    const float nrm = sqrtf(nn);
+    const float ux = vx / nrm, uy = vy / nrm;
+    const float inc = fabsf(ux * dx + uy * dy);
+    const float err = -inc + 1.0f;
+    return err < tol;
+}
+
+__device__ __forceinline__ bool inlier_test(float vx, float vy, float dx, float dy, float tol) {
+    const float nn = __builtin_fmaf(vx, vx, vy * vy);
+    const float dot = __builtin_fmaf(vx, dx, vy * dy);
+    const float e = 1.0f - fabsf(dot) * __builtin_amdgcn_rsqf(nn);
+    bool in = e < tol - kErrBand;
+    const bool sure = (in || e > tol + kErrBand) && nn > 1e-30f;
+    if (__builtin_expect(!sure, 0)) in = inlier_exact(vx, vy, dx, dy, tol);
+    return in;
+}
+
+struct Hyp {
+    float cx, cy, sub;
+    bool valid;
+};
+__device__ __forceinline__ Hyp make_hyp(const PencilSoA& m, uint32_t a, uint32_t b, float degeneracy_tol) {
+    const float hax = m.hx[a], hay = m.hy[a], haz = m.hz[a];
+    const float hbx = m.hx[b], hby = m.hy[b], hbz = m.hz[b];
+    const float ex = hax - hbx, ey = hay - hby, ez = haz - hbz;
+    const float dist = sqrtf((ex * ex + ey * ey) + ez * ez);
+    Hyp h;
+    h.valid = dist > degeneracy_tol;
+    const float px = hay * hbz - haz * hby;
+    const float py = haz * hbx - hax * hbz;
+    const float pz = hax * hby - hay * hbx;
+    const bool ideal = fabsf(pz) < kEps;
+    h.cx = ideal ? px : px / pz;
+    h.cy = ideal ? py : py / pz;
+    h.sub = ideal ? 0.f : 1.f;
+    return h;
+}
+__device__ __forceinline__ void hyp_v(const Hyp& h, float ax, float ay, float& vx, float& vy) {
+    vx = h.sub != 0.f ? h.cx - ax : h.cx;
+    vy = h.sub != 0.f ? h.cy - ay : h.cy;
+}
+
+constexpr float kTiny = 1e-30f;
+struct EstConst {
+    float k_in, k_out;
+};
+__device__ __forceinline__ EstConst est_const(float tol) {
+    const float a = (1.0f - tol) + kErrBand, b = (1.0f - tol) - kErrBand;
+    return EstConst{a * a, b * b};
+}
+typedef float f2 __attribute__((ext_vector_type(2)));
+__device__ __forceinline__ void inlier_estimate2(const f2 cx, const f2 cy, const f2 nsub, float ax, float ay, float dx, float dy,
+                                                 const EstConst& K, uint64_t& m_in0, uint64_t& m_un0, uint64_t& m_in1,
+                                                 uint64_t& m_un1) {
+    const f2 vx = __builtin_elementwise_fma(nsub, (f2){ax, ax}, cx), vy = __builtin_elementwise_fma(nsub, (f2){ay, ay}, cy);
+    const f2 nn = __builtin_elementwise_fma(vx, vx, vy * vy);
+    const f2 dot = __builtin_elementwise_fma(vx, (f2){dx, dx}, vy * (f2){dy, dy});
+    const f2 dd = dot * dot;
+    const f2 t_in = __builtin_elementwise_fma(nn, (f2){K.k_in, K.k_in}, (f2){kTiny, kTiny});
+    const f2 t_out = __builtin_elementwise_fma(nn, (f2){K.k_out, K.k_out}, (f2){-kTiny, -kTiny});
+    m_in0 = __builtin_amdgcn_fcmpf(dd.x, t_in.x, 2);
+    m_in1 = __builtin_amdgcn_fcmpf(dd.y, t_in.y, 2);
+    m_un0 = ~(m_in0 | __builtin_amdgcn_fcmpf(dd.x, t_out.x, 4));
+    m_un1 = ~(m_in1 | __builtin_amdgcn_fcmpf(dd.y, t_out.y, 4));
+}
+
+constexpr int kScoreChunk = 512;
+constexpr int kScoreTabFloats = 2 * 5 * kScoreChunk;
+template <int kH, int kThreads>
+__device__ __forceinline__ unsigned long long score_block(const PencilSoA& m, uint32_t n, uint32_t round, float tol,
+                                                          float degeneracy_tol, uint32_t n_iter, uint64_t seed,
+                                                          float* __restrict__ s_tab_, unsigned long long* __restrict__ s_key) {
+    float(*s_tab)[5][kScoreChunk] = reinterpret_cast<float(*)[5][kScoreChunk]>(s_tab_);
+    constexpr int kW = kThreads / 64;
+    const int lane = threadIdx.x & 63;
+    const uint32_t hyp0 = (blockIdx.x * kW + (threadIdx.x >> 6)) * kH;
+    float cx[kH], cy[kH], nsub[kH];
+    bool valid[kH];
+#pragma unroll
+    for (int j = 0; j < kH; ++j) {
+        uint32_t a, b;
+        sample_pair(seed, round, min(hyp0 + (uint32_t)j, n_iter - 1u), n, a, b);
+        const Hyp h = make_hyp(m, a, b, degeneracy_tol);
+        cx[j] = h.cx;
+        cy[j] = h.cy;
+        nsub[j] = -h.sub;
+        valid[j] = h.valid;
+    }
+    const EstConst K = est_const(tol);
+    float acc[kH];
+#pragma unroll
+    for (int j = 0; j < kH; ++j) acc[j] = 0.f;
+    auto stage = [&](int buf, uint32_t c0) {
+        for (uint32_t t = threadIdx.x; t < (uint32_t)kScoreChunk; t += kThreads) {
+            const uint32_t i = c0 + t;
+            if (i < n) {
+                s_tab[buf][0][t] = m.ax[i];
+                s_tab[buf][1][t] = m.ay[i];
+                s_tab[buf][2][t] = m.dx[i];
+                s_tab[buf][3][t] = m.dy[i];
+                s_tab[buf][4][t] = m.len[i];
+            }
+        }
+    };
+    stage(0, 0u);
+    int buf = 0;
+    for (uint32_t c0 = 0; c0 < n; c0 += kScoreChunk, buf ^= 1) {
+        __syncthreads();
+        if (c0 + kScoreChunk < n) stage(buf ^ 1, c0 + kScoreChunk);
+        const uint32_t cn = min((uint32_t)kScoreChunk, n - c0);
+        for (uint32_t t = lane; t < cn; t += 64) {
+            const float ax = s_tab[buf][0][t], ay = s_tab[buf][1][t], dx = s_tab[buf][2][t], dy = s_tab[buf][3][t];
+            const float len = s_tab[buf][4][t];
+            uint64_t any_unsure = 0ull, mu[kH];
+            static_assert(kH % 2 == 0, "hypotheses are scored in pairs");
+#pragma unroll
+            for (int j = 0; j < kH; j += 2) {
+                uint64_t mi0, mi1;
+                inlier_estimate2((f2){cx[j], cx[j + 1]}, (f2){cy[j], cy[j + 1]}, (f2){nsub[j], nsub[j + 1]}, ax, ay, dx, dy, K, mi0,
+                                 mu[j], mi1, mu[j + 1]);
+                acc[j] = acc[j] + (__builtin_amdgcn_inverse_ballot_w64(mi0 & ~mu[j]) ? len : 0.0f);
+                acc[j + 1] = acc[j + 1] + (__builtin_amdgcn_inverse_ballot_w64(mi1 & ~mu[j + 1]) ? len : 0.0f);
+                any_unsure |= mu[j] | mu[j + 1];
+            }
+            if (__builtin_expect(any_unsure != 0ull, 0)) {
+#pragma unroll
+                for (int j = 0; j < kH; ++j)
+                    if (__builtin_amdgcn_inverse_ballot_w64(mu[j])) {
+                        const float vx = __builtin_fmaf(nsub[j], ax, cx[j]), vy = __builtin_fmaf(nsub[j], ay, cy[j]);
+                        acc[j] = acc[j] + (inlier_exact(vx, vy, dx, dy, tol) ? len : 0.0f);
+                    }
+            }
+        }
+    }
+    unsigned long long key = 0ull;
+#pragma unroll
+    for (int j = 0; j < kH; ++j) {
+        const float score = wave_tree(acc[j]);
+        const uint32_t it = hyp0 + (uint32_t)j;
+        if (valid[j] && it < n_iter && score > 0.0f) {
+            const unsigned long long k = ((unsigned long long)__float_as_uint(score) << 32) | (unsigned long long)(0xFFFFFFFFu - it);
+            key = k > key ? k : key;
+        }
+    }
+    if (lane == 0) s_key[threadIdx.x >> 6] = key;
+    __syncthreads();
+    if (threadIdx.x == 0)
+        for (int wv = 1; wv < kW; ++wv) key = s_key[wv] > key ? s_key[wv] : key;
+    return key;
+}
+
+}
+}
```
